# Amandaynzhou/CGC-Net

Measured on AMD Instinct MI355X. Metric: cell-graphs/sec (fwd+bwd), batch=32, ~1800 nodes/16 feat, higher is better.
Workload: dtype f32

## Files before the change

cgc-net_amd/csrc/rowops.hip:

```cpp
#include <type_traits>

#include "common.hpp"
#include "groups.hpp"

#define L2_EPS 1e-12f
#define RENORM_EPS 1e-15f
#define MAX_SLOTS 1024

template <int VEC, int MAXJ, int NQ>
__device__ __forceinline__ void col_reduce_store(float (&acc)[NQ][MAXJ][VEC], int F, int lpr, float* smem, float* slot) {
  const int lane = threadIdx.x & 63, wave = threadIdx.x >> 6;
#pragma unroll
  for (int q = 0; q < NQ; ++q)
#pragma unroll
    for (int j = 0; j < MAXJ; ++j)
#pragma unroll
      for (int v = 0; v < VEC; ++v)
        for (int o = 32; o >= lpr; o >>= 1) acc[q][j][v] += __shfl_xor(acc[q][j][v], o);
  if (wave > 0 && lane < lpr) {
#pragma unroll
    for (int q = 0; q < NQ; ++q)
#pragma unroll
      for (int j = 0; j < MAXJ; ++j)
#pragma unroll
        for (int v = 0; v < VEC; ++v) {
          const int c = (lane + lpr * j) * VEC + v;
          if (c < F) smem[((wave - 1) * NQ + q) * F + c] = acc[q][j][v];
        }
  }
  __syncthreads();
  if (wave == 0 && lane < lpr) {
#pragma unroll
    for (int q = 0; q < NQ; ++q)
#pragma unroll
      for (int j = 0; j < MAXJ; ++j)
#pragma unroll
        for (int v = 0; v < VEC; ++v) {
          const int c = (lane + lpr * j) * VEC + v;
          if (c < F) {
            float t = acc[q][j][v];
            for (int w = 0; w < 3; ++w) t += smem[(w * NQ + q) * F + c];
            slot[q * F + c] = t;
          }
        }
  }
}

template <int VEC, int MAXJ>
__device__ __forceinline__ void col_reduce_store_f64(double (&acc)[2][MAXJ][VEC], int F, int lpr, double* smem, double* slot) {
  const int lane = threadIdx.x & 63, wave = threadIdx.x >> 6;
#pragma unroll
  for (int q = 0; q < 2; ++q) {
#pragma unroll
    for (int j = 0; j < MAXJ; ++j)
#pragma unroll
      for (int v = 0; v < VEC; ++v)
        for (int o = 32; o >= lpr; o >>= 1) acc[q][j][v] += __shfl_xor(acc[q][j][v], o);
    if (q > 0) __syncthreads();
    if (wave > 0 && lane < lpr) {
#pragma unroll
      for (int j = 0; j < MAXJ; ++j)
#pragma unroll
        for (int v = 0; v < VEC; ++v) {
          const int c = (lane + lpr * j) * VEC + v;
          if (c < F) smem[(wave - 1) * F + c] = acc[q][j][v];
        }
    }
    __syncthreads();
    if (wave == 0 && lane < lpr) {
#pragma unroll
      for (int j = 0; j < MAXJ; ++j)
#pragma unroll
        for (int v = 0; v < VEC; ++v) {
          const int c = (lane + lpr * j) * VEC + v;
          if (c < F) {
            double t = acc[q][j][v];
            for (int w = 0; w < 3; ++w) t += smem[w * F + c];
            slot[q * F + c] = t;
          }
        }
    }
  }
}

#define RS_GROUPS 32
template <typename OUT, typename IN = float>
__global__ __launch_bounds__(32 * RS_GROUPS) void k_reduce_slots(const IN* __restrict__ ws, int slots, int width, OUT* __restrict__ out) {
  __shared__ double part[RS_GROUPS][32];
  const int cl = threadIdx.x & 31, grp = threadIdx.x >> 5;
  const int c = blockIdx.x * 32 + cl;
  double s = 0.0;
  if (c < width) {
    double a[4] = {0.0, 0.0, 0.0, 0.0};
    int k = grp;
    for (; k + 3 * RS_GROUPS < slots; k += 4 * RS_GROUPS) {
#pragma unroll
      for (int u = 0; u < 4; ++u) a[u] += (double)ws[(size_t)(k + RS_GROUPS * u) * width + c];
    }
    for (; k < slots; k += RS_GROUPS) a[0] += (double)ws[(size_t)k * width + c];
    s = (a[0] + a[1]) + (a[2] + a[3]);
  }
  part[grp][cl] = s;
  __syncthreads();
  if (grp == 0 && c < width) {
    double t[4] = {0.0, 0.0, 0.0, 0.0};
#pragma unroll
    for (int g = 0; g < RS_GROUPS; g += 4) { t[0] += part[g][cl]; t[1] += part[g + 1][cl]; t[2] += part[g + 2][cl]; t[3] += part[g + 3][cl]; }
    out[c] = (OUT)((t[0] + t[1]) + (t[2] + t[3]));
  }
}
#define REDUCE_SLOTS_GRID(width) dim3(ceil_div((width), 32))

__global__ __launch_bounds__(32 * RS_GROUPS) void k_reduce_slots_pair(const float* __restrict__ ws0, float* __restrict__ out0,
                                                                     const float* __restrict__ ws1, float* __restrict__ out1, int slots, int width) {
  const float* __restrict__ ws = blockIdx.y ? ws1 : ws0;
  float* __restrict__ out = blockIdx.y ? out1 : out0;
  __shared__ double part[RS_GROUPS][32];
  const int cl = threadIdx.x & 31, grp = threadIdx.x >> 5;
  const int c = blockIdx.x * 32 + cl;
  double s = 0.0;
  if (c < width) {
    double a[4] = {0.0, 0.0, 0.0, 0.0};
    int k = grp;
    for (; k + 3 * RS_GROUPS < slots; k += 4 * RS_GROUPS) {
#pragma unroll
      for (int u = 0; u < 4; ++u) a[u] += (double)ws[(size_t)(k + RS_GROUPS * u) * width + c];
    }
    for (; k < slots; k += RS_GROUPS) a[0] += (double)ws[(size_t)k * width + c];
    s = (a[0] + a[1]) + (a[2] + a[3]);
  }
  part[grp][cl] = s;
  __syncthreads();
  if (grp == 0 && c < width) {
    double t[4] = {0.0, 0.0, 0.0, 0.0};
#pragma unroll
    for (int g = 0; g < RS_GROUPS; g += 4) { t[0] += part[g][cl]; t[1] += part[g + 1][cl]; t[2] += part[g + 2][cl]; t[3] += part[g + 3][cl]; }
    out[c] = (float)((t[0] + t[1]) + (t[2] + t[3]));
  }
}
int launch_reduce_slots_f32_pair(const float* ws0, float* out0, const float* ws1, float* out1, int ng, int slots, int width, hipStream_t stream) {
  hipLaunchKernelGGL(k_reduce_slots_pair, dim3(ceil_div(width, 32), ng), dim3(32 * RS_GROUPS), 0, stream, ws0, out0, ws1, out1, slots, width);
  CGC_RETURN_IF_LAUNCH_FAILED();
  return 0;
}

int launch_reduce_slots_f32(const float* ws, int slots, int width, float* out, hipStream_t stream) {
  hipLaunchKernelGGL(k_reduce_slots<float>, REDUCE_SLOTS_GRID(width), dim3(32 * RS_GROUPS), 0, stream, ws, slots, width, out);
  CGC_RETURN_IF_LAUNCH_FAILED();
  return 0;
}

struct ColCfg {
  int vec, maxj, lpr, blocks;
  bool ok;
};
static ColCfg col_cfg(int n, int F, bool vec_ok) {
  ColCfg c;
  c.vec = vec_ok ? 4 : 1;
  c.ok = true;
  int chunks = F / c.vec;
  if (chunks <= 64) {
    c.maxj = 1;
    c.lpr = pick_lpr(chunks);
  } else {
    c.lpr = 64;
    int need = ceil_div(chunks, 64);
    if (c.vec == 4 && need > 8) {
      c.vec = 1;
      need = ceil_div(F, 64);
    }
    c.ok = need <= 32;
    c.maxj = need <= 2 ? 2 : need <= 4 ? 4 : (need == 5 && c.vec == 4) ? 5 : need <= 8 ? 8 : need <= 16 ? 16 : 32;
  }
  c.blocks = row_blocks(n, c.lpr, MAX_SLOTS);
  return c;
}

#define DISPATCH_COL(KERNEL, cfg, smem_bytes, stream, ...)                                                   \
  do {                                                                                                       \
    dim3 g__((cfg).blocks), b__(CGC_BLOCK);                                                                  \
    if ((cfg).vec == 4) {                                                                                    \
      switch ((cfg).maxj) {                                                                                  \
        case 1: hipLaunchKernelGGL((KERNEL<4, 1>), g__, b__, smem_bytes, stream, __VA_ARGS__); break;        \
        case 2: hipLaunchKernelGGL((KERNEL<4, 2>), g__, b__, smem_bytes, stream, __VA_ARGS__); break;        \
        case 4: hipLaunchKernelGGL((KERNEL<4, 4>), g__, b__, smem_bytes, stream, __VA_ARGS__); break;        \
        case 5: hipLaunchKernelGGL((KERNEL<4, 5>), g__, b__, smem_bytes, stream, __VA_ARGS__); break;        \
        default: hipLaunchKernelGGL((KERNEL<4, 8>), g__, b__, smem_bytes, stream, __VA_ARGS__); break;       \
      }                                                                                                      \
    } else {                                                                                                 \
      switch ((cfg).maxj) {                                                                                  \
        case 1: hipLaunchKernelGGL((KERNEL<1, 1>), g__, b__, smem_bytes, stream, __VA_ARGS__); break;        \
        case 2: hipLaunchKernelGGL((KERNEL<1, 2>), g__, b__, smem_bytes, stream, __VA_ARGS__); break;        \
        case 4: hipLaunchKernelGGL((KERNEL<1, 4>), g__, b__, smem_bytes, stream, __VA_ARGS__); break;        \
        case 8: hipLaunchKernelGGL((KERNEL<1, 8>), g__, b__, smem_bytes, stream, __VA_ARGS__); break;        \
        case 16: hipLaunchKernelGGL((KERNEL<1, 16>), g__, b__, smem_bytes, stream, __VA_ARGS__); break;      \
        default: hipLaunchKernelGGL((KERNEL<1, 32>), g__, b__, smem_bytes, stream, __VA_ARGS__); break;      \
      }                                                                                                      \
    }                                                                                                        \
  } while (0)

#define DISPATCH_COL_Y(KERNEL, cfg, ny, smem_bytes, stream, ...)                                                   \
  do {                                                                                                       \
    dim3 g__((cfg).blocks, (ny)), b__(CGC_BLOCK);                                                                    \
    if ((cfg).vec == 4) {                                                                                    \
      switch ((cfg).maxj) {                                                                                  \
        case 1: hipLaunchKernelGGL((KERNEL<4, 1>), g__, b__, smem_bytes, stream, __VA_ARGS__); break;        \
        case 2: hipLaunchKernelGGL((KERNEL<4, 2>), g__, b__, smem_bytes, stream, __VA_ARGS__); break;        \
        case 4: hipLaunchKernelGGL((KERNEL<4, 4>), g__, b__, smem_bytes, stream, __VA_ARGS__); break;        \
        case 5: hipLaunchKernelGGL((KERNEL<4, 5>), g__, b__, smem_bytes, stream, __VA_ARGS__); break;        \
        default: hipLaunchKernelGGL((KERNEL<4, 8>), g__, b__, smem_bytes, stream, __VA_ARGS__); break;       \
      }                                                                                                      \
    } else {                                                                                                 \
      switch ((cfg).maxj) {                                                                                  \
        case 1: hipLaunchKernelGGL((KERNEL<1, 1>), g__, b__, smem_bytes, stream, __VA_ARGS__); break;        \
        case 2: hipLaunchKernelGGL((KERNEL<1, 2>), g__, b__, smem_bytes, stream, __VA_ARGS__); break;        \
        case 4: hipLaunchKernelGGL((KERNEL<1, 4>), g__, b__, smem_bytes, stream, __VA_ARGS__); break;        \
        case 8: hipLaunchKernelGGL((KERNEL<1, 8>), g__, b__, smem_bytes, stream, __VA_ARGS__); break;        \
        case 16: hipLaunchKernelGGL((KERNEL<1, 16>), g__, b__, smem_bytes, stream, __VA_ARGS__); break;      \
        default: hipLaunchKernelGGL((KERNEL<1, 32>), g__, b__, smem_bytes, stream, __VA_ARGS__); break;      \
      }                                                                                                      \
    }                                                                                                        \
  } while (0)


extern "C" int cgc_stats_blocks(int n, int F) {
  (void)F;
  int b = ceil_div(n > 0 ? n : 1, 4);
  return b < MAX_SLOTS ? b : MAX_SLOTS;
}
extern "C" int64_t cgc_stats_ws_floats(int n, int F) {
  const int b = cgc_stats_blocks(n, F);
  return (int64_t)(b > 1 ? b : 1) * 4 * F + 4 * (int64_t)F + 2;
}

template <int VEC, int MAXJ>
__global__ __launch_bounds__(256) void k_l2norm_act_stats(const float* __restrict__ h, int n, int F, int lpr, int normalize,
                                                          int act, float* __restrict__ hn, float* __restrict__ rinv,
                                                          float* __restrict__ ws) {
  extern __shared__ __attribute__((aligned(16))) float smem[];
  const RowGroup rg(lpr);
  double acc[2][MAXJ][VEC];
#pragma unroll
  for (int j = 0; j < MAXJ; ++j)
#pragma unroll
    for (int v = 0; v < VEC; ++v) acc[0][j][v] = acc[1][j][v] = 0.0;

  for (int base = rg.gwave * rg.rpw; base < n; base += rg.nwaves * rg.rpw) {
    const int row = base + rg.sub;
    const bool valid = row < n;
    Vec<VEC> x[MAXJ];
    float ss = 0.f;
#pragma unroll
    for (int j = 0; j < MAXJ; ++j) {
      const int c = (rg.sl + lpr * j) * VEC;
      if (valid && c < F) {
        load_wide<VEC, MAXJ>(x[j], h + (size_t)row * F + c);
#pragma unroll
        for (int v = 0; v < VEC; ++v) ss += x[j].v[v] * x[j].v[v];
      } else {
#pragma unroll
        for (int v = 0; v < VEC; ++v) x[j].v[v] = 0.f;
      }
    }
    ss = group_sum(ss, lpr);
    const float r = normalize ? 1.f / fmaxf(sqrtf(ss), L2_EPS) : 1.f;
#pragma unroll
    for (int j = 0; j < MAXJ; ++j) {
      const int c = (rg.sl + lpr * j) * VEC;
      if (valid && c < F) {
#pragma unroll
        for (int v = 0; v < VEC; ++v) {
          x[j].v[v] *= r;
          const double o = (double)act_fwd(x[j].v[v], act);
          acc[0][j][v] += o;
          acc[1][j][v] = fma(o, o, acc[1][j][v]);
        }
        x[j].store(hn + (size_t)row * F + c);
      }
    }
    if (valid && rg.sl == 0) rinv[row] = r;
  }
  if (ws != nullptr)
    col_reduce_store_f64<VEC, MAXJ>(acc, F, lpr, reinterpret_cast<double*>(smem), reinterpret_cast<double*>(ws) + (size_t)blockIdx.x * 2 * F);
}

extern "C" int cgc_l2norm_act_stats(const float* h, int n, int F, int normalize, int act, float* hn, float* rinv,
                                    double* stats, float* ws, cgc_stream_t stream) {
  if (n <= 0 || F <= 0) {
    if (stats && F > 0) (void)hipMemsetAsync(stats, 0, sizeof(double) * 2 * F, as_stream(stream));
    return 0;
  }
  const bool vec_ok = (F % 4 == 0) && aligned16(h) && aligned16(hn);
  ColCfg cfg = col_cfg(n, F, vec_ok);
  if (!cfg.ok) return CGC_EINVAL;
  float* wsp = stats ? ws : nullptr;
  if (stats && !ws) return CGC_EINVAL;
  const size_t smem = sizeof(float) * 3 * 2 * F;
  DISPATCH_COL(k_l2norm_act_stats, cfg, smem, as_stream(stream), h, n, F, cfg.lpr, normalize, act, hn, rinv, wsp);
  CGC_RETURN_IF_LAUNCH_FAILED();
  if (stats) {
    hipLaunchKernelGGL((k_reduce_slots<double, double>), REDUCE_SLOTS_GRID(2 * F), dim3(32 * RS_GROUPS), 0, as_stream(stream),
                       reinterpret_cast<const double*>(ws), cfg.blocks, 2 * F, stats);
    CGC_RETURN_IF_LAUNCH_FAILED();
  }
  return 0;
}

__global__ void k_bn_finalize(const double* __restrict__ stats, int F, double count, float eps, float momentum,
                              float* running_mean, float* running_var, float* __restrict__ mean, float* __restrict__ istd,
                              long long* nbt) {
  const int f = blockIdx.x * blockDim.x + threadIdx.x;
  if (f == 0 && nbt != nullptr) *nbt += 1;
  if (f >= F) return;
  const double m = stats[f] / count;
  double var = stats[F + f] / count - m * m;
  if (var < 0.0) var = 0.0;
  mean[f] = (float)m;
  istd[f] = (float)(1.0 / sqrt(var + (double)eps));
  if (running_mean != nullptr) {
    const double unbiased = var * count / (count > 1.0 ? count - 1.0 : 1.0);
    running_mean[f] = (1.f - momentum) * running_mean[f] + momentum * (float)m;
    running_var[f] = (1.f - momentum) * running_var[f] + momentum * (float)unbiased;
  }
}

extern "C" int cgc_bn_finalize(const double* stats, int F, double count, float eps, float momentum, float* running_mean,
                               float* running_var, float* mean, float* istd, cgc_stream_t stream) {
  if (F <= 0) return 0;
  hipLaunchKernelGGL(k_bn_finalize, dim3(ceil_div(F, 256)), dim3(256), 0, as_stream(stream), stats, F, count, eps, momentum,
                     running_mean, running_var, mean, istd, (long long*)nullptr);
  CGC_RETURN_IF_LAUNCH_FAILED();
  return 0;
}

__global__ void k_bn_running_stats(const float* __restrict__ rm, const float* __restrict__ rv, int F, float eps, float* __restrict__ mean,
                                   float* __restrict__ istd) {
  const int f = blockIdx.x * blockDim.x + threadIdx.x;
  if (f >= F) return;
  mean[f] = rm[f];
  istd[f] = 1.f / sqrtf(rv[f] + eps);
}
extern "C" int cgc_bn_running_stats(const float* running_mean, const float* running_var, int F, float eps, float* mean, float* istd,
                                    cgc_stream_t stream) {
  if (F <= 0) return 0;
  if (running_mean == nullptr || running_var == nullptr || mean == nullptr || istd == nullptr) return CGC_EINVAL;
  hipLaunchKernelGGL(k_bn_running_stats, dim3(ceil_div(F, 256)), dim3(256), 0, as_stream(stream), running_mean, running_var, F, eps, mean, istd);
  CGC_RETURN_IF_LAUNCH_FAILED();
  return 0;
}

__global__ __launch_bounds__(32 * RS_GROUPS) void k_stats_finalize(const StatsFinPtrs p0, const StatsFinPtrs p1, int slots, int F, double count) {
  const StatsFinPtrs& p = blockIdx.y ? p1 : p0;
  const double* __restrict__ ws = reinterpret_cast<const double*>(p.ws);
  const float eps = p.eps, momentum = p.momentum;
  float* running_mean = p.running_mean;
  float* running_var = p.running_var;
  float* __restrict__ mean = p.mean;
  float* __restrict__ istd = p.istd;
  long long* nbt = p.nbt;
  __shared__ double part[2][RS_GROUPS][32];
  const int cl = threadIdx.x & 31, grp = threadIdx.x >> 5;
  const int f = blockIdx.x * 32 + cl;
  if (blockIdx.x == 0 && threadIdx.x == 0 && nbt != nullptr) *nbt += 1;
#pragma unroll
  for (int q = 0; q < 2; ++q) {
    double s = 0.0;
    if (f < F) {
      const double* col = ws + (size_t)q * F + f;
      const size_t width = 2 * (size_t)F;
      double a[4] = {0.0, 0.0, 0.0, 0.0};
      int k = grp;
      for (; k + 3 * RS_GROUPS < slots; k += 4 * RS_GROUPS) {
#pragma unroll
        for (int u = 0; u < 4; ++u) a[u] += col[(size_t)(k + RS_GROUPS * u) * width];
      }
      for (; k < slots; k += RS_GROUPS) a[0] += col[(size_t)k * width];
      s = (a[0] + a[1]) + (a[2] + a[3]);
    }
    part[q][grp][cl] = s;
  }
  __syncthreads();
  if (grp != 0 || f >= F) return;
  double t0[4] = {0.0, 0.0, 0.0, 0.0}, t1[4] = {0.0, 0.0, 0.0, 0.0};
#pragma unroll
  for (int g = 0; g < RS_GROUPS; g += 4)
#pragma unroll
    for (int u = 0; u < 4; ++u) { t0[u] += part[0][g + u][cl]; t1[u] += part[1][g + u][cl]; }
  const double s0 = (t0[0] + t0[1]) + (t0[2] + t0[3]), s1 = (t1[0] + t1[1]) + (t1[2] + t1[3]);
  const double m = s0 / count;
  double var = s1 / count - m * m;
  if (var < 0.0) var = 0.0;
  mean[f] = (float)m;
  istd[f] = (float)(1.0 / sqrt(var + (double)eps));
  if (running_mean != nullptr) {
    const double unbiased = var * count / (count > 1.0 ? count - 1.0 : 1.0);
    running_mean[f] = (1.f - momentum) * running_mean[f] + momentum * (float)m;
    running_var[f] = (1.f - momentum) * running_var[f] + momentum * (float)unbiased;
  }
}

int launch_stats_finalize_groups(const StatsFinPtrs* g, int ng, int slots, int F, double count, hipStream_t stream) {
  hipLaunchKernelGGL(k_stats_finalize, dim3(ceil_div(F, 32), ng), dim3(32 * RS_GROUPS), 0, stream, g[0], g[ng - 1], slots, F, count);
  CGC_RETURN_IF_LAUNCH_FAILED();
  return 0;
}
int launch_stats_finalize(const float* ws, int slots, int F, double count, float eps, float momentum, float* running_mean,
                          float* running_var, float* mean, float* istd, int64_t* nbt, hipStream_t stream) {
  const StatsFinPtrs g{ws, running_mean, running_var, mean, istd, reinterpret_cast<long long*>(nbt), eps, momentum};
  return launch_stats_finalize_groups(&g, 1, slots, F, count, stream);
}

extern "C" int cgc_l2norm_act_bn(const float* h, int n, int F, int normalize, int act, float* hn, float* rinv, float* ws,
                                 double count, float eps, float momentum, float* running_mean, float* running_var,
                                 int64_t* num_batches_tracked, float* mean, float* istd, cgc_stream_t stream) {
  if (F <= 0) return 0;
  if (ws == nullptr || mean == nullptr || istd == nullptr) return CGC_EINVAL;
  int slots = 0;
  if (n > 0) {
    const bool vec_ok = (F % 4 == 0) && aligned16(h) && aligned16(hn);
    ColCfg cfg = col_cfg(n, F, vec_ok);
    if (!cfg.ok) return CGC_EINVAL;
    const size_t smem = sizeof(float) * 3 * 2 * F;
    DISPATCH_COL(k_l2norm_act_stats, cfg, smem, as_stream(stream), h, n, F, cfg.lpr, normalize, act, hn, rinv, ws);
    CGC_RETURN_IF_LAUNCH_FAILED();
    slots = cfg.blocks;
  }
  return launch_stats_finalize(ws, slots, F, count, eps, momentum, running_mean, running_var, mean, istd, num_batches_tracked, as_stream(stream));
}

template <int VEC, int MAXJ>
__global__ __launch_bounds__(256) void k_bn_act_apply(const BnApplyPtrs p0, const BnApplyPtrs p1, int n, int F, int lpr, int act, int ldy) {
  const BnApplyPtrs& p = blockIdx.y ? p1 : p0;
  const float* __restrict__ hn = p.hn;
  const float* __restrict__ mean = p.mean;
  const float* __restrict__ istd = p.istd;
  const float* __restrict__ gamma = p.gamma;
  const float* __restrict__ beta = p.beta;
  float* __restrict__ y = p.y;
  float* __restrict__ y2 = p.y2;
  const int ldy2 = p.ldy2;
  const RowGroup rg(lpr);
  float mu[MAXJ][VEC], sc[MAXJ][VEC], sh[MAXJ][VEC];
#pragma unroll
  for (int j = 0; j < MAXJ; ++j)
#pragma unroll
    for (int v = 0; v < VEC; ++v) {
      mu[j][v] = 0.f;
      sc[j][v] = 1.f;
      sh[j][v] = 0.f;
    }
  if (mean != nullptr) {
#pragma unroll
    for (int j = 0; j < MAXJ; ++j)
#pragma unroll
      for (int v = 0; v < VEC; ++v) {
        const int c = min((rg.sl + lpr * j) * VEC + v, F - 1);
        mu[j][v] = mean[c];
        sc[j][v] = istd[c] * gamma[c];
        sh[j][v] = beta[c];
      }
  }
  auto rows = [&](auto act_c) {
    constexpr int ACT = decltype(act_c)::value;
    const int last = F - VEC;
    for (int base = rg.gwave * rg.rpw; base < n; base += rg.nwaves * rg.rpw) {
      const int row = base + rg.sub;
      const bool rowok = row < n;
      Vec<VEC> x[MAXJ];
#pragma unroll
      for (int j = 0; j < MAXJ; ++j) load_wide<VEC, MAXJ>(x[j], hn + (size_t)min(row, n - 1) * F + min((rg.sl + lpr * j) * VEC, last));
#pragma unroll
      for (int j = 0; j < MAXJ; ++j) {
        const int c = (rg.sl + lpr * j) * VEC;
#pragma unroll
        for (int v = 0; v < VEC; ++v) x[j].v[v] = fmaf(act_fwd(x[j].v[v], ACT) - mu[j][v], sc[j][v], sh[j][v]);
        if (rowok && c < F) {
          x[j].store(y + (size_t)row * ldy + c);
          if (y2 != nullptr) x[j].store(y2 + (size_t)row * ldy2 + c);
        }
      }
    }
  };
  switch (act) {
    case CGC_ACT_RELU: rows(std::integral_constant<int, CGC_ACT_RELU>()); break;
    case CGC_ACT_ELU: rows(std::integral_constant<int, CGC_ACT_ELU>()); break;
    case CGC_ACT_LEAKYRELU: rows(std::integral_constant<int, CGC_ACT_LEAKYRELU>()); break;
    default: rows(std::integral_constant<int, CGC_ACT_IDENTITY>()); break;
  }
}

int bn_act_apply_groups(const BnApplyPtrs* g, int ng, int n, int F, int act, int ldy, hipStream_t stream) {
  if (n <= 0 || F <= 0) return 0;
  if (ng < 1 || ng > 2) return CGC_EINVAL;
  bool vec = (F % 4 == 0) && (ldy % 4 == 0);
  for (int i = 0; i < ng; ++i)
    vec = vec && aligned16(g[i].hn) && aligned16(g[i].y) && (g[i].y2 == nullptr || (g[i].ldy2 % 4 == 0 && aligned16(g[i].y2)));
  ColCfg cfg = col_cfg(n, F, vec);
  if (!cfg.ok) return CGC_EINVAL;
  cfg.blocks = row_blocks(n, cfg.lpr, 1024);
  DISPATCH_COL_Y(k_bn_act_apply, cfg, ng, 0, stream, g[0], g[ng - 1], n, F, cfg.lpr, act, ldy);
  CGC_RETURN_IF_LAUNCH_FAILED();
  return 0;
}
extern "C" int cgc_bn_act_apply(const float* hn, int n, int F, int act, const float* mean, const float* istd, const float* gamma,
                                const float* beta, float* y, int ldy, float* y2, int ldy2, cgc_stream_t stream) {
  const BnApplyPtrs g{hn, mean, istd, gamma, beta, y, y2, ldy2};
  return bn_act_apply_groups(&g, 1, n, F, act, ldy, as_stream(stream));
}

template <int VEC, int MAXJ>
__global__ __launch_bounds__(256) void k_bn_bwd_reduce(const BnRedPtrs p0, const BnRedPtrs p1, int ldy, int n, int F, int lpr, int act) {
  const BnRedPtrs& p = blockIdx.y ? p1 : p0;
  const float* __restrict__ dy = p.dy;
  const float* __restrict__ hn = p.hn;
  const float* __restrict__ mean = p.mean;
  const float* __restrict__ istd = p.istd;
  float* __restrict__ ws = p.ws;
  extern __shared__ __attribute__((aligned(16))) float smem[];
  const RowGroup rg(lpr);
  float acc[2][MAXJ][VEC];
  float mu[MAXJ][VEC], is[MAXJ][VEC];
#pragma unroll
  for (int j = 0; j < MAXJ; ++j)
#pragma unroll
    for (int v = 0; v < VEC; ++v) {
      acc[0][j][v] = acc[1][j][v] = 0.f;
      const int c = min((rg.sl + lpr * j) * VEC + v, F - 1);
      mu[j][v] = mean[c];
      is[j][v] = istd[c];
    }
  for (int base = rg.gwave * rg.rpw; base < n; base += rg.nwaves * rg.rpw) {
    const int row = base + rg.sub;
    if (row < n) {
#pragma unroll
      for (int j = 0; j < MAXJ; ++j) {
        const int c = (rg.sl + lpr * j) * VEC;
        if (c < F) {
          Vec<VEC> d, x;
          load_wide<VEC, MAXJ>(d, dy + (size_t)row * ldy + c);
          load_wide<VEC, MAXJ>(x, hn + (size_t)row * F + c);
#pragma unroll
          for (int v = 0; v < VEC; ++v) {
            const float xhat = (act_fwd(x.v[v], act) - mu[j][v]) * is[j][v];
            acc[0][j][v] += d.v[v];
            acc[1][j][v] += d.v[v] * xhat;
          }
        }
      }
    }
  }
  col_reduce_store<VEC, MAXJ, 2>(acc, F, lpr, smem, ws + (size_t)blockIdx.x * 2 * F);
}

int bn_bwd_reduce_groups(const BnRedPtrs* g, float* const* sums, int ng, int ldy, int n, int F, int act, hipStream_t stream) {
  if (F <= 0) return 0;
  if (ng < 1 || ng > 2) return CGC_EINVAL;
  if (n <= 0) {
    for (int i = 0; i < ng; ++i) (void)hipMemsetAsync(sums[i], 0, sizeof(float) * 2 * F, stream);
    return 0;
  }
  bool vec_ok = (F % 4 == 0) && (ldy % 4 == 0);
  for (int i = 0; i < ng; ++i) vec_ok = vec_ok && aligned16(g[i].dy) && aligned16(g[i].hn);
  ColCfg cfg = col_cfg(n, F, vec_ok);
  if (!cfg.ok) return CGC_EINVAL;
  const size_t smem = sizeof(float) * 3 * 2 * F;
  DISPATCH_COL_Y(k_bn_bwd_reduce, cfg, ng, smem, stream, g[0], g[ng - 1], ldy, n, F, cfg.lpr, act);
  CGC_RETURN_IF_LAUNCH_FAILED();
  return launch_reduce_slots_f32_pair(g[0].ws, sums[0], g[ng - 1].ws, sums[ng - 1], ng, cfg.blocks, 2 * F, stream);
}
extern "C" int cgc_bn_bwd_reduce(const float* dy, int ldy, const float* hn, int n, int F, int act, const float* mean,
                                 const float* istd, float* sums, float* ws, cgc_stream_t stream) {
  const BnRedPtrs g{dy, hn, mean, istd, ws};
  float* const out[1] = {sums};
  return bn_bwd_reduce_groups(&g, out, 1, ldy, n, F, act, as_stream(stream));
}

template <int VEC, int MAXJ>
__global__ __launch_bounds__(256) void k_bn_act_l2_bwd(const float* __restrict__ dy, int ldy, const float* __restrict__ hn,
                                                       const float* __restrict__ rinv, int n, int F, int lpr, int act,
                                                       int normalize, int mode, const float* __restrict__ mean,
                                                       const float* __restrict__ istd, const float* __restrict__ gamma,
                                                       const float* __restrict__ sums, float inv_count, float* __restrict__ dh,
                                                       float* __restrict__ ws ) {
  extern __shared__ __attribute__((aligned(16))) float smem[];
  const RowGroup rg(lpr);
  float csum[1][MAXJ][VEC];
#pragma unroll
  for (int j = 0; j < MAXJ; ++j)
#pragma unroll
    for (int v = 0; v < VEC; ++v) csum[0][j][v] = 0.f;
  constexpr bool REGC = MAXJ * VEC <= 8;
  constexpr int RJ = REGC ? MAXJ : 1, RV = REGC ? VEC : 1;
  float ca[RJ][RV], cb[RJ][RV], cc[RJ][RV], mu[RJ][RV], is[RJ][RV];
  if (REGC) {
#pragma unroll
    for (int j = 0; j < RJ; ++j)
#pragma unroll
      for (int v = 0; v < RV; ++v) {
        const int c = (rg.sl + lpr * j) * VEC + v;
        ca[j][v] = 1.f; cb[j][v] = cc[j][v] = mu[j][v] = is[j][v] = 0.f;
        if (mode != 0 && c < F) {
          ca[j][v] = gamma[c] * istd[c];
          if (mode == 2) {
            cb[j][v] = ca[j][v] * sums[c] * inv_count;
            cc[j][v] = ca[j][v] * sums[F + c] * inv_count;
            mu[j][v] = mean[c];
            is[j][v] = istd[c];
          }
        }
      }
  }
  float* const lc = smem + 3 * (size_t)F;
  if (!REGC && mode != 0) {
    for (int c = threadIdx.x; c < F; c += blockDim.x) {
      const float a_ = gamma[c] * istd[c];
      lc[c] = a_;
      lc[F + c] = mode == 2 ? a_ * sums[c] * inv_count : 0.f;
      lc[2 * F + c] = mode == 2 ? a_ * sums[F + c] * inv_count : 0.f;
      lc[3 * F + c] = mode == 2 ? mean[c] : 0.f;
      lc[4 * F + c] = mode == 2 ? istd[c] : 0.f;
    }
    __syncthreads();
  }
  auto rows = [&](auto act_c, auto hot_c) {
    constexpr int ACT = decltype(act_c)::value;
    constexpr bool HOT = decltype(hot_c)::value;
    const int mode_rt = mode, normalize_rt = normalize;
    const int mode = HOT ? 2 : mode_rt;
    const int normalize = HOT ? 1 : normalize_rt;
    for (int base = rg.gwave * rg.rpw; base < n; base += rg.nwaves * rg.rpw) {
      const int row = min(base + rg.sub, n - 1);
      const bool valid = base + rg.sub < n;
      Vec<VEC> g[MAXJ], x[MAXJ];
      float dot = 0.f;
  #pragma unroll
      for (int j = 0; j < MAXJ; ++j) {
        const int c = min((rg.sl + lpr * j) * VEC, F - VEC);
        load_wide<VEC, MAXJ>(g[j], dy + (size_t)row * ldy + c);
        load_wide<VEC, MAXJ>(x[j], hn + (size_t)row * F + c);
      }
  #pragma unroll
      for (int j = 0; j < MAXJ; ++j) {
        const int c = (rg.sl + lpr * j) * VEC;
        if (valid && c < F) {
          Vec<VEC> pa, pb, pc, pm, pi;
          if (!REGC && mode != 0) {
            pa.load(lc + c);
            if (mode == 2) { pb.load(lc + F + c); pc.load(lc + 2 * F + c); pm.load(lc + 3 * F + c); pi.load(lc + 4 * F + c); }
          }
  #pragma unroll
          for (int v = 0; v < VEC; ++v) {
            const float xv = x[j].v[v];
            float a_, b_ = 0.f, c_ = 0.f, m_ = 0.f, i_ = 0.f;
            if (REGC) {
              a_ = ca[REGC ? j : 0][REGC ? v : 0]; b_ = cb[REGC ? j : 0][REGC ? v : 0]; c_ = cc[REGC ? j : 0][REGC ? v : 0];
              m_ = mu[REGC ? j : 0][REGC ? v : 0]; i_ = is[REGC ? j : 0][REGC ? v : 0];
            } else if (mode != 0) {
              a_ = pa.v[v];
              if (mode == 2) { b_ = pb.v[v]; c_ = pc.v[v]; m_ = pm.v[v]; i_ = pi.v[v]; }
            } else {
              a_ = 1.f;
            }
            float go = a_ * g[j].v[v];
            if (mode == 2) go = go - b_ - (act_fwd(xv, ACT) - m_) * i_ * c_;
            go *= act_bwd(xv, ACT);
            g[j].v[v] = go;
            dot += xv * go;
          }
        } else {
  #pragma unroll
          for (int v = 0; v < VEC; ++v) g[j].v[v] = x[j].v[v] = 0.f;
        }
      }
      if (normalize) dot = group_sum(dot, lpr);
      if (!valid) continue;
      const float r = normalize ? rinv[row] : 1.f;
      const bool clamped = normalize && !(r < 1.f / L2_EPS);
  #pragma unroll
      for (int j = 0; j < MAXJ; ++j) {
        const int c = (rg.sl + lpr * j) * VEC;
        if (c < F) {
          Vec<VEC> o;
  #pragma unroll
          for (int v = 0; v < VEC; ++v) {
            const float gv = g[j].v[v];
            o.v[v] = !normalize ? gv : (clamped ? gv * (1.f / L2_EPS) : r * (gv - x[j].v[v] * dot));
            csum[0][j][v] += o.v[v];
          }
          o.store(dh + (size_t)row * F + c);
        }
      }
    }
  };
  if (mode == 2 && normalize) {
    switch (act) {
      case CGC_ACT_RELU: rows(std::integral_constant<int, CGC_ACT_RELU>(), std::true_type()); break;
      case CGC_ACT_ELU: rows(std::integral_constant<int, CGC_ACT_ELU>(), std::true_type()); break;
      case CGC_ACT_LEAKYRELU: rows(std::integral_constant<int, CGC_ACT_LEAKYRELU>(), std::true_type()); break;
      default: rows(std::integral_constant<int, CGC_ACT_IDENTITY>(), std::true_type()); break;
    }
  } else {
    switch (act) {
      case CGC_ACT_RELU: rows(std::integral_constant<int, CGC_ACT_RELU>(), std::false_type()); break;
      case CGC_ACT_ELU: rows(std::integral_constant<int, CGC_ACT_ELU>(), std::false_type()); break;
      case CGC_ACT_LEAKYRELU: rows(std::integral_constant<int, CGC_ACT_LEAKYRELU>(), std::false_type()); break;
      default: rows(std::integral_constant<int, CGC_ACT_IDENTITY>(), std::false_type()); break;
    }
  }
  if (ws != nullptr) col_reduce_store<VEC, MAXJ, 1>(csum, F, lpr, smem, ws + (size_t)blockIdx.x * F);
}

extern "C" int cgc_bn_act_l2_bwd(const float* dy, int ldy, const float* hn, const float* rinv, int n, int F, int act,
                                 int normalize, int mode, const float* mean, const float* istd, const float* gamma,
                                 const float* sums, double count, float* dh, float* dh_colsum, float* ws, cgc_stream_t stream) {
  if (F <= 0) return 0;
  if (n <= 0) {
    if (dh_colsum) (void)hipMemsetAsync(dh_colsum, 0, sizeof(float) * F, as_stream(stream));
    return 0;
  }
  if (dh_colsum != nullptr && ws == nullptr) return CGC_EINVAL;
  const bool vec = (F % 4 == 0) && (ldy % 4 == 0) && aligned16(dy) && aligned16(hn) && aligned16(dh);
  ColCfg cfg = col_cfg(n, F, vec);
  if (!cfg.ok) return CGC_EINVAL;
  if (dh_colsum == nullptr) cfg.blocks = row_blocks(n, cfg.lpr);
  const float inv_count = (float)(1.0 / count);
  const size_t smem = sizeof(float) * (3 + 5) * F;
  DISPATCH_COL(k_bn_act_l2_bwd, cfg, smem, as_stream(stream), dy, ldy, hn, rinv, n, F, cfg.lpr, act, normalize, mode, mean, istd,
               gamma, sums, inv_count, dh, dh_colsum ? ws : (float*)nullptr);
  CGC_RETURN_IF_LAUNCH_FAILED();
  if (dh_colsum) {
    hipLaunchKernelGGL(k_reduce_slots<float>, REDUCE_SLOTS_GRID(F), dim3(32 * RS_GROUPS), 0, as_stream(stream), ws, cfg.blocks, F, dh_colsum);
    CGC_RETURN_IF_LAUNCH_FAILED();
  }
  return 0;
}

template <int VEC, int MAXJ>
__global__ __launch_bounds__(256) void k_colsum(const float* __restrict__ x, int ld, int n, int F, int lpr, float* __restrict__ ws) {
  extern __shared__ __attribute__((aligned(16))) float smem[];
  const RowGroup rg(lpr);
  float acc[1][MAXJ][VEC];
#pragma unroll
  for (int j = 0; j < MAXJ; ++j)
#pragma unroll
    for (int v = 0; v < VEC; ++v) acc[0][j][v] = 0.f;
  for (int base = rg.gwave * rg.rpw; base < n; base += rg.nwaves * rg.rpw) {
    const int row = base + rg.sub;
    if (row < n) {
#pragma unroll
      for (int j = 0; j < MAXJ; ++j) {
        const int c = (rg.sl + lpr * j) * VEC;
        if (c < F) {
          Vec<VEC> d;
          d.load(x + (size_t)row * ld + c);
#pragma unroll
          for (int v = 0; v < VEC; ++v) acc[0][j][v] += d.v[v];
        }
      }
    }
  }
  col_reduce_store<VEC, MAXJ, 1>(acc, F, lpr, smem, ws + (size_t)blockIdx.x * F);
}

extern "C" int cgc_colsum(const float* x, int ld, int n, int F, float* out, float* ws, cgc_stream_t stream) {
  if (F <= 0) return 0;
  if (n <= 0) {
    (void)hipMemsetAsync(out, 0, sizeof(float) * F, as_stream(stream));
    return 0;
  }
  const bool vec_ok = (F % 4 == 0) && (ld % 4 == 0) && aligned16(x);
  ColCfg cfg = col_cfg(n, F, vec_ok);
  if (!cfg.ok) return CGC_EINVAL;
  const size_t smem = sizeof(float) * 3 * F;
  DISPATCH_COL(k_colsum, cfg, smem, as_stream(stream), x, ld, n, F, cfg.lpr, ws);
  CGC_RETURN_IF_LAUNCH_FAILED();
  hipLaunchKernelGGL(k_reduce_slots<float>, REDUCE_SLOTS_GRID(F), dim3(32 * RS_GROUPS), 0, as_stream(stream), ws, cfg.blocks, F, out);
  CGC_RETURN_IF_LAUNCH_FAILED();
  return 0;
}

template <int VEC>
__global__ __launch_bounds__(256) void k_softmax_fwd(const float* __restrict__ x, int n, int C, int ld, int lpr, float* __restrict__ out) {
  const RowGroup rg(lpr);
  for (int base = rg.gwave * rg.rpw; base < n; base += rg.nwaves * rg.rpw) {
    const int row = base + rg.sub;
    const bool valid = row < n;
    const float* xr = x + (size_t)row * ld;
    float m = -INFINITY;
    if (valid)
      for (int c = rg.sl * VEC; c < C; c += lpr * VEC) {
        Vec<VEC> t;
        t.load(xr + c);
#pragma unroll
        for (int v = 0; v < VEC; ++v) m = fmaxf(m, t.v[v]);
      }
    m = group_max(m, lpr);
    float s = 0.f;
    if (valid)
      for (int c = rg.sl * VEC; c < C; c += lpr * VEC) {
        Vec<VEC> t;
        t.load(xr + c);
#pragma unroll
        for (int v = 0; v < VEC; ++v) s += expf(t.v[v] - m);
      }
    s = group_sum(s, lpr);
    if (!valid) continue;
    const float inv = 1.f / s;
    for (int c = rg.sl * VEC; c < C; c += lpr * VEC) {
      Vec<VEC> t;
      t.load(xr + c);
#pragma unroll
      for (int v = 0; v < VEC; ++v) t.v[v] = expf(t.v[v] - m) * inv;
      t.store(out + (size_t)row * ld + c);
    }
  }
}

template <int VEC, int MAXJ>
__global__ __launch_bounds__(256) void k_softmax_fwd_reg(const float* __restrict__ x, int n, int C, int ld, int lpr,
                                                         float* __restrict__ out) {
  const RowGroup rg(lpr);
  for (int base = rg.gwave * rg.rpw; base < n; base += rg.nwaves * rg.rpw) {
    const int row = base + rg.sub;
    const bool valid = row < n;
    const float* xr = x + (size_t)row * ld;
    Vec<VEC> t[MAXJ];
    float m = -INFINITY;
#pragma unroll
    for (int j = 0; j < MAXJ; ++j) {
      const int c = (rg.sl + lpr * j) * VEC;
      if (valid && c < C) {
        t[j].load(xr + c);
#pragma unroll
        for (int v = 0; v < VEC; ++v) m = fmaxf(m, t[j].v[v]);
      }
    }
    m = group_max(m, lpr);
    float s = 0.f;
#pragma unroll
    for (int j = 0; j < MAXJ; ++j) {
      const int c = (rg.sl + lpr * j) * VEC;
      if (valid && c < C) {
#pragma unroll
        for (int v = 0; v < VEC; ++v) {
          t[j].v[v] = expf(t[j].v[v] - m);
          s += t[j].v[v];
        }
      }
    }
    s = group_sum(s, lpr);
    if (!valid) continue;
    const float inv = 1.f / s;
#pragma unroll
    for (int j = 0; j < MAXJ; ++j) {
      const int c = (rg.sl + lpr * j) * VEC;
      if (c < C) {
#pragma unroll
        for (int v = 0; v < VEC; ++v) t[j].v[v] *= inv;
        t[j].store(out + (size_t)row * ld + c);
      }
    }
  }
}

template <int VEC, int MAXJ>
__global__ __launch_bounds__(256) void k_softmax_bwd(const float* __restrict__ S, const float* __restrict__ dS, int n, int C,
                                                     int ld, int lpr, float* __restrict__ dx, float* __restrict__ ws) {
  extern __shared__ __attribute__((aligned(16))) float smem[];
  const RowGroup rg(lpr);
  float csum[1][MAXJ][VEC];
#pragma unroll
  for (int j = 0; j < MAXJ; ++j)
#pragma unroll
    for (int v = 0; v < VEC; ++v) csum[0][j][v] = 0.f;
  for (int base = rg.gwave * rg.rpw; base < n; base += rg.nwaves * rg.rpw) {
    const int row = min(base + rg.sub, n - 1);
    const bool valid = base + rg.sub < n;
    Vec<VEC> s[MAXJ], d[MAXJ];
    float dot = 0.f;
#pragma unroll
    for (int j = 0; j < MAXJ; ++j) {
      const int c = min((rg.sl + lpr * j) * VEC, C - VEC);
      load_wide<VEC, MAXJ>(s[j], S + (size_t)row * ld + c);
      load_wide<VEC, MAXJ>(d[j], dS + (size_t)row * ld + c);
    }
#pragma unroll
    for (int j = 0; j < MAXJ; ++j) {
      const bool ok = valid && (rg.sl + lpr * j) * VEC < C;
#pragma unroll
      for (int v = 0; v < VEC; ++v) {
        s[j].v[v] = ok ? s[j].v[v] : 0.f;
        d[j].v[v] = ok ? d[j].v[v] : 0.f;
        dot += s[j].v[v] * d[j].v[v];
      }
    }
    dot = group_sum(dot, lpr);
    if (!valid) continue;
#pragma unroll
    for (int j = 0; j < MAXJ; ++j) {
      const int c = (rg.sl + lpr * j) * VEC;
      if (c < C) {
#pragma unroll
        for (int v = 0; v < VEC; ++v) {
          d[j].v[v] = s[j].v[v] * (d[j].v[v] - dot);
          csum[0][j][v] += d[j].v[v];
        }
        d[j].store(dx + (size_t)row * ld + c);
      }
    }
  }
  if (ws != nullptr) col_reduce_store<VEC, MAXJ, 1>(csum, C, lpr, smem, ws + (size_t)blockIdx.x * C);
}

extern "C" int cgc_softmax_fwd(const float* x, int n, int C, int ld, float* out, cgc_stream_t stream) {
  if (n <= 0 || C <= 0) return 0;
  if (ld < C) return CGC_EINVAL;
  const bool vec = (C % 4 == 0) && (ld % 4 == 0) && aligned16(x) && aligned16(out);
  ColCfg cfg = col_cfg(n, C, vec);
  if (cfg.ok && cfg.maxj <= 8) {
    cfg.blocks = row_blocks(n, cfg.lpr);
    DISPATCH_COL(k_softmax_fwd_reg, cfg, 0, as_stream(stream), x, n, C, ld, cfg.lpr, out);
    CGC_RETURN_IF_LAUNCH_FAILED();
    return 0;
  }
  const int lpr = pick_lpr(vec ? C / 4 : C);
  dim3 grid(row_blocks(n, lpr)), block(CGC_BLOCK);
  if (vec)
    hipLaunchKernelGGL(k_softmax_fwd<4>, grid, block, 0, as_stream(stream), x, n, C, ld, lpr, out);
  else
    hipLaunchKernelGGL(k_softmax_fwd<1>, grid, block, 0, as_stream(stream), x, n, C, ld, lpr, out);
  CGC_RETURN_IF_LAUNCH_FAILED();
  return 0;
}

extern "C" int cgc_softmax_bwd(const float* S, const float* dS, int n, int C, int ld, float* dx, float* dx_colsum, float* ws,
                               cgc_stream_t stream) {
  if (C <= 0) return 0;
  if (ld < C) return CGC_EINVAL;
  if (n <= 0) {
    if (dx_colsum) (void)hipMemsetAsync(dx_colsum, 0, sizeof(float) * C, as_stream(stream));
    return 0;
  }
  if (dx_colsum != nullptr && ws == nullptr) return CGC_EINVAL;
  const bool vec = (C % 4 == 0) && (ld % 4 == 0) && aligned16(S) && aligned16(dS) && aligned16(dx);
  ColCfg cfg = col_cfg(n, C, vec);
  if (!cfg.ok) return CGC_EINVAL;
  if (dx_colsum == nullptr) cfg.blocks = row_blocks(n, cfg.lpr);
  const size_t smem = dx_colsum ? sizeof(float) * 3 * C : 0;
  DISPATCH_COL(k_softmax_bwd, cfg, smem, as_stream(stream), S, dS, n, C, ld, cfg.lpr, dx, dx_colsum ? ws : (float*)nullptr);
  CGC_RETURN_IF_LAUNCH_FAILED();
  if (dx_colsum) {
    hipLaunchKernelGGL(k_reduce_slots<float>, REDUCE_SLOTS_GRID(C), dim3(32 * RS_GROUPS), 0, as_stream(stream), ws, cfg.blocks, C, dx_colsum);
    CGC_RETURN_IF_LAUNCH_FAILED();
  }
  return 0;
}

#define SEGMAX_WAVES 16
__global__ __launch_bounds__(64 * SEGMAX_WAVES) void k_segment_max_fwd(const float* __restrict__ x, const int* __restrict__ gptr,
                                                                       int D, int nmax, float* __restrict__ out,
                                                                       int* __restrict__ arg) {
  __shared__ float bv[SEGMAX_WAVES][64];
  __shared__ int bi[SEGMAX_WAVES][64];
  const int b = blockIdx.x;
  const int lane = threadIdx.x & 63, wave = threadIdx.x >> 6;
  int dp = 64;
  if (D <= 32) dp = D <= 2 ? 2 : D <= 4 ? 4 : D <= 8 ? 8 : D <= 16 ? 16 : 32;
  const int rpw = 64 / dp, sub = lane / dp, dl = lane - sub * dp;
  const int d = blockIdx.y * 64 + dl;
  const int lo = gptr[b], hi = gptr[b + 1];
  float best = -INFINITY;
  int idx = -1;
  if (d < D) {
    const int stride = SEGMAX_WAVES * rpw;
    int r = lo + wave * rpw + sub;
    for (; r + 3 * stride < hi; r += 4 * stride) {
      float v[4];
#pragma unroll
      for (int u = 0; u < 4; ++u) v[u] = x[(size_t)(r + u * stride) * D + d];
#pragma unroll
      for (int u = 0; u < 4; ++u)
        if (v[u] > best) { best = v[u]; idx = r + u * stride; }
    }
    for (; r < hi; r += stride) {
      const float v = x[(size_t)r * D + d];
      if (v > best) { best = v; idx = r; }
    }
  }
  bv[wave][lane] = best;
  bi[wave][lane] = idx;
  __syncthreads();
  if (wave == 0 && sub == 0 && d < D) {
    for (int w = 0; w < SEGMAX_WAVES; ++w)
      for (int s2 = (w == 0 ? 1 : 0); s2 < rpw; ++s2) {
        const float v = bv[w][s2 * dp + dl];
        const int i = bi[w][s2 * dp + dl];
        if (i >= 0 && (v > best || (v == best && i < idx) || idx < 0)) { best = v; idx = i; }
      }
    if (idx < 0) { best = 0.f; }
    else if (hi - lo < nmax && best < 0.f) { best = 0.f; idx = -1; }
    out[(size_t)b * D + d] = best;
    arg[(size_t)b * D + d] = idx;
  }
}

__global__ void k_segment_max_bwd(const float* __restrict__ dout, const int* __restrict__ arg, int total, int D, float* __restrict__ dx) {
  const int i = blockIdx.x * blockDim.x + threadIdx.x;
  if (i >= total) return;
  const int a = arg[i];
  if (a >= 0) dx[(size_t)a * D + (i % D)] = dout[i];
}

extern "C" int cgc_segment_max_fwd(const float* x, const int* gptr, int B, int D, int nmax, float* out, int* arg, cgc_stream_t stream) {
  if (B <= 0 || D <= 0) return 0;
  hipLaunchKernelGGL(k_segment_max_fwd, dim3(B, ceil_div(D, 64)), dim3(64 * SEGMAX_WAVES), 0, as_stream(stream), x, gptr, D, nmax, out, arg);
  CGC_RETURN_IF_LAUNCH_FAILED();
  return 0;
}

__global__ void k_segment_max_bwd_full(const float* __restrict__ dout, const int* __restrict__ arg, const int* __restrict__ gptr, int D,
                                       float* __restrict__ dx) {
  const int b = blockIdx.y;
  const int g0 = gptr[b], cnt = (gptr[b + 1] - g0) * D;
  for (int i = blockIdx.x * blockDim.x + threadIdx.x; i < cnt; i += gridDim.x * blockDim.x) {
    const int r = i / D, d = i - r * D;
    dx[(size_t)g0 * D + i] = (arg[b * D + d] == g0 + r) ? dout[b * D + d] : 0.f;
  }
}

extern "C" int cgc_segment_max_bwd_full(const float* dout, const int* arg, const int* gptr, int B, int D, int nmax, float* dx,
                                        cgc_stream_t stream) {
  if (B <= 0 || D <= 0 || nmax <= 0) return 0;
  if (B > 65535) return CGC_EINVAL;
  int bx = ceil_div(nmax * D, 256 * 4);
  if (bx < 1) bx = 1;
  hipLaunchKernelGGL(k_segment_max_bwd_full, dim3(bx, B), dim3(256), 0, as_stream(stream), dout, arg, gptr, D, dx);
  CGC_RETURN_IF_LAUNCH_FAILED();
  return 0;
}

extern "C" int cgc_segment_max_bwd(const float* dout, const int* arg, int B, int D, float* dx_zeroed, cgc_stream_t stream) {
  if (B <= 0 || D <= 0) return 0;
  const int total = B * D;
  hipLaunchKernelGGL(k_segment_max_bwd, dim3(ceil_div(total, 256)), dim3(256), 0, as_stream(stream), dout, arg, total, D, dx_zeroed);
  CGC_RETURN_IF_LAUNCH_FAILED();
  return 0;
}

template <int VEC>
__global__ __launch_bounds__(256) void k_dense_rownorm_fwd(const float* __restrict__ A, int R, int C, int lpr, float* __restrict__ out,
                                                           float* __restrict__ invd, float* __restrict__ ge1) {
  const RowGroup rg(lpr);
  for (int base = rg.gwave * rg.rpw; base < R; base += rg.nwaves * rg.rpw) {
    const int row = base + rg.sub;
    const bool valid = row < R;
    float s = 0.f;
    if (valid)
      for (int c = rg.sl * VEC; c < C; c += lpr * VEC) {
        Vec<VEC> t;
        t.load(A + (size_t)row * C + c);
#pragma unroll
        for (int v = 0; v < VEC; ++v) s += t.v[v];
      }
    s = group_sum(s, lpr);
    if (!valid) continue;
    const float inv = 1.f / fmaxf(s, 1.f);
    for (int c = rg.sl * VEC; c < C; c += lpr * VEC) {
      Vec<VEC> t;
      t.load(A + (size_t)row * C + c);
#pragma unroll
      for (int v = 0; v < VEC; ++v) t.v[v] *= inv;
      t.store(out + (size_t)row * C + c);
    }
    if (rg.sl == 0) {
      invd[row] = inv;
      ge1[row] = s >= 1.f ? 1.f : 0.f;
    }
  }
}

template <int VEC>
__global__ __launch_bounds__(256) void k_dense_rownorm_bwd(const float* __restrict__ dOut, const float* __restrict__ An,
                                                           const float* __restrict__ invd, const float* __restrict__ ge1, int R, int C,
                                                           int lpr, float* __restrict__ dA) {
  const RowGroup rg(lpr);
  for (int base = rg.gwave * rg.rpw; base < R; base += rg.nwaves * rg.rpw) {
    const int row = base + rg.sub;
    const bool valid = row < R;
    float t = 0.f;
    if (valid)
      for (int c = rg.sl * VEC; c < C; c += lpr * VEC) {
        Vec<VEC> g, a;
        g.load(dOut + (size_t)row * C + c);
        a.load(An + (size_t)row * C + c);
#pragma unroll
        for (int v = 0; v < VEC; ++v) t += g.v[v] * a.v[v];
      }
    t = group_sum(t, lpr);
    if (!valid) continue;
    const float inv = invd[row], sub = ge1[row] * t;
    for (int c = rg.sl * VEC; c < C; c += lpr * VEC) {
      Vec<VEC> g;
      g.load(dOut + (size_t)row * C + c);
#pragma unroll
      for (int v = 0; v < VEC; ++v) g.v[v] = inv * (g.v[v] - sub);
      g.store(dA + (size_t)row * C + c);
    }
  }
}

template <int VEC>
__global__ __launch_bounds__(256) void k_dense_renorm_fwd(const float* __restrict__ A, int R, int C, int lpr, float p, float* __restrict__ out) {
  const RowGroup rg(lpr);
  const float omp = 1.f - p;
  for (int base = rg.gwave * rg.rpw; base < R; base += rg.nwaves * rg.rpw) {
    const int row = base + rg.sub;
    const bool valid = row < R;
    const int diag = valid ? row % C : -1;
    float s = 0.f;
    if (valid)
      for (int c = rg.sl * VEC; c < C; c += lpr * VEC) {
        Vec<VEC> t;
        t.load(A + (size_t)row * C + c);
#pragma unroll
        for (int v = 0; v < VEC; ++v) s += (c + v == diag) ? 0.f : t.v[v];
      }
    s = group_sum(s, lpr);
    if (!valid) continue;
    const float den = s + RENORM_EPS;
    for (int c = rg.sl * VEC; c < C; c += lpr * VEC) {
      Vec<VEC> t;
      t.load(A + (size_t)row * C + c);
#pragma unroll
      for (int v = 0; v < VEC; ++v) t.v[v] = (c + v == diag) ? p : (t.v[v] / den) * omp;
      t.store(out + (size_t)row * C + c);
    }
  }
}

template <int VEC>
__global__ __launch_bounds__(256) void k_dense_renorm_bwd(const float* __restrict__ A, const float* __restrict__ dOut, int R, int C,
                                                          int lpr, float p, float* __restrict__ dA) {
  const RowGroup rg(lpr);
  const float omp = 1.f - p;
  for (int base = rg.gwave * rg.rpw; base < R; base += rg.nwaves * rg.rpw) {
    const int row = base + rg.sub;
    const bool valid = row < R;
    const int diag = valid ? row % C : -1;
    float s = 0.f, t = 0.f;
    if (valid)
      for (int c = rg.sl * VEC; c < C; c += lpr * VEC) {
        Vec<VEC> a, g;
        a.load(A + (size_t)row * C + c);
        g.load(dOut + (size_t)row * C + c);
#pragma unroll
        for (int v = 0; v < VEC; ++v)
          if (c + v != diag) { s += a.v[v]; t += a.v[v] * g.v[v]; }
      }
    s = group_sum(s, lpr);
    t = group_sum(t, lpr);
    if (!valid) continue;
    const float q = 1.f / (s + RENORM_EPS);
    for (int c = rg.sl * VEC; c < C; c += lpr * VEC) {
      Vec<VEC> g;
      g.load(dOut + (size_t)row * C + c);
#pragma unroll
      for (int v = 0; v < VEC; ++v) g.v[v] = (c + v == diag) ? 0.f : omp * q * (g.v[v] - q * t);
      g.store(dA + (size_t)row * C + c);
    }
  }
}

template <int VEC>
__global__ __launch_bounds__(256) void k_adj_prep_fwd(const float* __restrict__ A, int R, int C, int lpr, float p, float* __restrict__ At,
                                                      float* __restrict__ An, float* __restrict__ invd, float* __restrict__ ge1) {
  const RowGroup rg(lpr);
  const bool renorm = p >= 0.f;
  const float omp = 1.f - p;
  for (int base = rg.gwave * rg.rpw; base < R; base += rg.nwaves * rg.rpw) {
    const int row = base + rg.sub;
    const bool valid = row < R;
    const int diag = (valid && renorm) ? row % C : -1;
    float s = 0.f;
    if (valid)
      for (int c = rg.sl * VEC; c < C; c += lpr * VEC) {
        Vec<VEC> t;
        t.load(A + (size_t)row * C + c);
#pragma unroll
        for (int v = 0; v < VEC; ++v) s += (c + v == diag) ? 0.f : t.v[v];
      }
    s = group_sum(s, lpr);
    float st = s;
    const float den = s + RENORM_EPS;
    if (renorm) {
      st = 0.f;
      if (valid)
        for (int c = rg.sl * VEC; c < C; c += lpr * VEC) {
          Vec<VEC> t;
          t.load(A + (size_t)row * C + c);
#pragma unroll
          for (int v = 0; v < VEC; ++v) { t.v[v] = (c + v == diag) ? p : (t.v[v] / den) * omp; st += t.v[v]; }
          t.store(At + (size_t)row * C + c);
        }
      st = group_sum(st, lpr);
    }
    if (!valid) continue;
    const float inv = 1.f / fmaxf(st, 1.f);
    for (int c = rg.sl * VEC; c < C; c += lpr * VEC) {
      Vec<VEC> t;
      t.load(A + (size_t)row * C + c);
#pragma unroll
      for (int v = 0; v < VEC; ++v) {
        const float at = renorm ? ((c + v == diag) ? p : (t.v[v] / den) * omp) : t.v[v];
        t.v[v] = at * inv;
      }
      t.store(An + (size_t)row * C + c);
    }
    if (rg.sl == 0) {
      invd[row] = inv;
      ge1[row] = st >= 1.f ? 1.f : 0.f;
    }
  }
}

template <int VEC>
__global__ __launch_bounds__(256) void k_adj_prep_bwd(const float* __restrict__ A, const float* __restrict__ An, const float* __restrict__ invd,
                                                      const float* __restrict__ ge1, const float* __restrict__ gAn,
                                                      const float* __restrict__ gAt, int R, int C, int lpr, float p, float* __restrict__ dA) {
  const RowGroup rg(lpr);
  const bool renorm = p >= 0.f;
  const float omp = 1.f - p;
  for (int base = rg.gwave * rg.rpw; base < R; base += rg.nwaves * rg.rpw) {
    const int row = base + rg.sub;
    const bool valid = row < R;
    const int diag = (valid && renorm) ? row % C : -1;
    float t1 = 0.f, s = 0.f, u = 0.f, w = 0.f;
    if (valid)
      for (int c = rg.sl * VEC; c < C; c += lpr * VEC) {
        Vec<VEC> g, an, a, h;
        g.load(gAn + (size_t)row * C + c);
        an.load(An + (size_t)row * C + c);
#pragma unroll
        for (int v = 0; v < VEC; ++v) t1 += g.v[v] * an.v[v];
        if (renorm) {
          a.load(A + (size_t)row * C + c);
          if (gAt != nullptr) h.load(gAt + (size_t)row * C + c);
#pragma unroll
          for (int v = 0; v < VEC; ++v)
            if (c + v != diag) { s += a.v[v]; u += a.v[v] * g.v[v]; if (gAt != nullptr) w += a.v[v] * h.v[v]; }
        }
      }
    t1 = group_sum(t1, lpr);
    if (renorm) { s = group_sum(s, lpr); u = group_sum(u, lpr); w = group_sum(w, lpr); }
    if (!valid) continue;
    const float inv = invd[row], sub = ge1[row] * t1;
    const float q = 1.f / (s + RENORM_EPS);
    const float t = inv * (u - sub * s) + w;
    for (int c = rg.sl * VEC; c < C; c += lpr * VEC) {
      Vec<VEC> g, h;
      g.load(gAn + (size_t)row * C + c);
      if (gAt != nullptr) h.load(gAt + (size_t)row * C + c);
#pragma unroll
      for (int v = 0; v < VEC; ++v) {
        float d = inv * (g.v[v] - sub);
        if (gAt != nullptr) d += h.v[v];
        g.v[v] = renorm ? ((c + v == diag) ? 0.f : omp * q * (d - q * t)) : d;
      }
      g.store(dA + (size_t)row * C + c);
    }
  }
}

template <int VEC, int MAXJ>
__global__ __launch_bounds__(256) void k_adj_prep_fwd_reg(const float* __restrict__ A, int R, int C, int lpr, float p, float* __restrict__ At,
                                                          float* __restrict__ An, float* __restrict__ invd, float* __restrict__ ge1) {
  const RowGroup rg(lpr);
  const bool renorm = p >= 0.f;
  const float omp = 1.f - p;
  for (int base = rg.gwave * rg.rpw; base < R; base += rg.nwaves * rg.rpw) {
    const int row = base + rg.sub;
    const bool valid = row < R;
    const int diag = (valid && renorm) ? row % C : -1;
    Vec<VEC> t[MAXJ];
    float s = 0.f;
#pragma unroll
    for (int j = 0; j < MAXJ; ++j) {
      const int c = (rg.sl + lpr * j) * VEC;
      if (valid && c < C) {
        t[j].load(A + (size_t)row * C + c);
#pragma unroll
        for (int v = 0; v < VEC; ++v) s += (c + v == diag) ? 0.f : t[j].v[v];
      }
    }
    s = group_sum(s, lpr);
    float st = s;
    const float den = s + RENORM_EPS;
    if (renorm) {
      st = 0.f;
#pragma unroll
      for (int j = 0; j < MAXJ; ++j) {
        const int c = (rg.sl + lpr * j) * VEC;
        if (valid && c < C) {
#pragma unroll
          for (int v = 0; v < VEC; ++v) { t[j].v[v] = (c + v == diag) ? p : (t[j].v[v] / den) * omp; st += t[j].v[v]; }
          t[j].store(At + (size_t)row * C + c);
        }
      }
      st = group_sum(st, lpr);
    }
    if (!valid) continue;
    const float inv = 1.f / fmaxf(st, 1.f);
#pragma unroll
    for (int j = 0; j < MAXJ; ++j) {
      const int c = (rg.sl + lpr * j) * VEC;
      if (c < C) {
#pragma unroll
        for (int v = 0; v < VEC; ++v) t[j].v[v] *= inv;
        t[j].store(An + (size_t)row * C + c);
      }
    }
    if (rg.sl == 0) {
      invd[row] = inv;
      ge1[row] = st >= 1.f ? 1.f : 0.f;
    }
  }
}

template <int VEC, int MAXJ>
__global__ __launch_bounds__(256) void k_adj_prep_bwd_reg(const float* __restrict__ A, const float* __restrict__ An,
                                                          const float* __restrict__ invd, const float* __restrict__ ge1,
                                                          const float* __restrict__ gAn, const float* __restrict__ gAt, int R, int C,
                                                          int lpr, float p, float* __restrict__ dA) {
  const RowGroup rg(lpr);
  const bool renorm = p >= 0.f;
  const float omp = 1.f - p;
  for (int base = rg.gwave * rg.rpw; base < R; base += rg.nwaves * rg.rpw) {
    const int row = base + rg.sub;
    const bool valid = row < R;
    const int diag = (valid && renorm) ? row % C : -1;
    float t1 = 0.f, s = 0.f, u = 0.f, w = 0.f;
    Vec<VEC> g[MAXJ], h[MAXJ];
    if (renorm) {
      Vec<VEC> a[MAXJ];
#pragma unroll
      for (int j = 0; j < MAXJ; ++j) {
        const int c = (rg.sl + lpr * j) * VEC;
        if (valid && c < C) {
          load_wide<VEC, MAXJ>(g[j], gAn + (size_t)row * C + c);
          load_wide<VEC, MAXJ>(a[j], A + (size_t)row * C + c);
          if (gAt != nullptr) load_wide<VEC, MAXJ>(h[j], gAt + (size_t)row * C + c);
#pragma unroll
          for (int v = 0; v < VEC; ++v) s += (c + v == diag) ? 0.f : a[j].v[v];
        }
      }
      s = group_sum(s, lpr);
      const float den = s + RENORM_EPS, inv_f = valid ? invd[row] : 0.f;
#pragma unroll
      for (int j = 0; j < MAXJ; ++j) {
        const int c = (rg.sl + lpr * j) * VEC;
        if (valid && c < C) {
#pragma unroll
          for (int v = 0; v < VEC; ++v) {
            const bool dg = c + v == diag;
            const float at = dg ? p : (a[j].v[v] / den) * omp;
            t1 += g[j].v[v] * (at * inv_f);
            if (!dg) { u += a[j].v[v] * g[j].v[v]; if (gAt != nullptr) w += a[j].v[v] * h[j].v[v]; }
          }
        }
      }
    } else {
#pragma unroll
      for (int j = 0; j < MAXJ; ++j) {
        const int c = (rg.sl + lpr * j) * VEC;
        if (valid && c < C) {
          Vec<VEC> an;
          load_wide<VEC, MAXJ>(g[j], gAn + (size_t)row * C + c);
          load_wide<VEC, MAXJ>(an, An + (size_t)row * C + c);
#pragma unroll
          for (int v = 0; v < VEC; ++v) t1 += g[j].v[v] * an.v[v];
          if (gAt != nullptr) load_wide<VEC, MAXJ>(h[j], gAt + (size_t)row * C + c);
        }
      }
    }
    t1 = group_sum(t1, lpr);
    if (renorm) { u = group_sum(u, lpr); w = group_sum(w, lpr); }
    if (!valid) continue;
    const float inv = invd[row], sub = ge1[row] * t1;
    const float q = 1.f / (s + RENORM_EPS);
    const float t = inv * (u - sub * s) + w;
#pragma unroll
    for (int j = 0; j < MAXJ; ++j) {
      const int c = (rg.sl + lpr * j) * VEC;
      if (c < C) {
#pragma unroll
        for (int v = 0; v < VEC; ++v) {
          float d = inv * (g[j].v[v] - sub);
          if (gAt != nullptr) d += h[j].v[v];
          g[j].v[v] = renorm ? ((c + v == diag) ? 0.f : omp * q * (d - q * t)) : d;
        }
        g[j].store(dA + (size_t)row * C + c);
      }
    }
  }
}

#define LAUNCH_ROW(KERNEL, vec, lpr, R, stream, ...)                                                          \
  do {                                                                                                        \
    dim3 g__(row_blocks(R, lpr)), b__(CGC_BLOCK);                                                             \
    if (vec) hipLaunchKernelGGL(KERNEL<4>, g__, b__, 0, stream, __VA_ARGS__);                                 \
    else hipLaunchKernelGGL(KERNEL<1>, g__, b__, 0, stream, __VA_ARGS__);                                     \
  } while (0)

extern "C" int cgc_dense_rownorm_fwd(const float* A, int R, int C, float* out, float* invd, float* ge1, cgc_stream_t stream) {
  if (R <= 0 || C <= 0) return 0;
  const bool vec = (C % 4 == 0) && aligned16(A) && aligned16(out);
  const int lpr = pick_lpr(vec ? C / 4 : C);
  LAUNCH_ROW(k_dense_rownorm_fwd, vec, lpr, R, as_stream(stream), A, R, C, lpr, out, invd, ge1);
  CGC_RETURN_IF_LAUNCH_FAILED();
  return 0;
}
extern "C" int cgc_dense_rownorm_bwd(const float* dOut, const float* Anorm, const float* invd, const float* ge1, int R, int C,
                                     float* dA, cgc_stream_t stream) {
  if (R <= 0 || C <= 0) return 0;
  const bool vec = (C % 4 == 0) && aligned16(dOut) && aligned16(Anorm) && aligned16(dA);
  const int lpr = pick_lpr(vec ? C / 4 : C);
  LAUNCH_ROW(k_dense_rownorm_bwd, vec, lpr, R, as_stream(stream), dOut, Anorm, invd, ge1, R, C, lpr, dA);
  CGC_RETURN_IF_LAUNCH_FAILED();
  return 0;
}
extern "C" int cgc_dense_renorm_fwd(const float* A, int R, int C, float p, float* out, cgc_stream_t stream) {
  if (R <= 0 || C <= 0) return 0;
  const bool vec = (C % 4 == 0) && aligned16(A) && aligned16(out);
  const int lpr = pick_lpr(vec ? C / 4 : C);
  LAUNCH_ROW(k_dense_renorm_fwd, vec, lpr, R, as_stream(stream), A, R, C, lpr, p, out);
  CGC_RETURN_IF_LAUNCH_FAILED();
  return 0;
}
extern "C" int cgc_dense_renorm_bwd(const float* A, const float* dOut, int R, int C, float p, float* dA, cgc_stream_t stream) {
  if (R <= 0 || C <= 0) return 0;
  const bool vec = (C % 4 == 0) && aligned16(A) && aligned16(dOut) && aligned16(dA);
  const int lpr = pick_lpr(vec ? C / 4 : C);
  LAUNCH_ROW(k_dense_renorm_bwd, vec, lpr, R, as_stream(stream), A, dOut, R, C, lpr, p, dA);
  CGC_RETURN_IF_LAUNCH_FAILED();
  return 0;
}

extern "C" int cgc_adj_prep_fwd(const float* A, int R, int C, float p, float* At, float* An, float* invd, float* ge1, cgc_stream_t stream) {
  if (R <= 0 || C <= 0) return 0;
  if (p >= 0.f && At == nullptr) return CGC_EINVAL;
  const bool vec = (C % 4 == 0) && aligned16(A) && aligned16(An) && (At == nullptr || aligned16(At));
  ColCfg cfg = col_cfg(R, C, vec);
  if (cfg.ok && cfg.maxj <= 8) {
    cfg.blocks = row_blocks(R, cfg.lpr);
    DISPATCH_COL(k_adj_prep_fwd_reg, cfg, 0, as_stream(stream), A, R, C, cfg.lpr, p, At, An, invd, ge1);
    CGC_RETURN_IF_LAUNCH_FAILED();
    return 0;
  }
  const int lpr = pick_lpr(vec ? C / 4 : C);
  LAUNCH_ROW(k_adj_prep_fwd, vec, lpr, R, as_stream(stream), A, R, C, lpr, p, At, An, invd, ge1);
  CGC_RETURN_IF_LAUNCH_FAILED();
  return 0;
}
extern "C" int cgc_adj_prep_bwd(const float* A, const float* An, const float* invd, const float* ge1, const float* gAn, const float* gAt,
                                int R, int C, float p, float* dA, cgc_stream_t stream) {
  if (R <= 0 || C <= 0) return 0;
  const bool vec = (C % 4 == 0) && aligned16(A) && aligned16(An) && aligned16(gAn) && aligned16(dA) && (gAt == nullptr || aligned16(gAt));
  ColCfg cfg = col_cfg(R, C, vec);
  if (cfg.ok && cfg.maxj <= 8) {
    cfg.blocks = row_blocks(R, cfg.lpr);
    DISPATCH_COL(k_adj_prep_bwd_reg, cfg, 0, as_stream(stream), A, An, invd, ge1, gAn, gAt, R, C, cfg.lpr, p, dA);
    CGC_RETURN_IF_LAUNCH_FAILED();
    return 0;
  }
  const int lpr = pick_lpr(vec ? C / 4 : C);
  LAUNCH_ROW(k_adj_prep_bwd, vec, lpr, R, as_stream(stream), A, An, invd, ge1, gAn, gAt, R, C, lpr, p, dA);
  CGC_RETURN_IF_LAUNCH_FAILED();
  return 0;
}
```

cgc-net_amd/csrc/sagenarrow.hip:

```cpp
#include "common.hpp"
#include "groups.hpp"

#define L2_EPS 1e-12f
typedef float floatx16 __attribute__((ext_vector_type(16)));

template <int CTRL>
__device__ __forceinline__ float dpp_step(float v) {
  return v + __builtin_bit_cast(float, __builtin_amdgcn_mov_dpp(__builtin_bit_cast(int, v), CTRL, 0xF, 0xF, true));
}
__device__ __forceinline__ float half_sum(float v) {
  v = dpp_step<0xB1>(v);
  v = dpp_step<0x4E>(v);
  v = dpp_step<0x141>(v);
  v = dpp_step<0x140>(v);
  return v + __shfl_xor(v, 16);
}

#define SN_LDT 33

template <int FS, int ACT>
__global__ __launch_bounds__(256) void k_sage_narrow_bwd(const SnBwdPtrs p0, const SnBwdPtrs p1, int ldy, int n, int F, int ,
                                                         int normalize, int mode, float inv_count, int lda, int fin, int ldd, int tiles) {
  const bool second = blockIdx.y != 0;
  const float* __restrict__ dy = second ? p1.dy : p0.dy;
  const float* __restrict__ hn = second ? p1.hn : p0.hn;
  const float* __restrict__ rinv = second ? p1.rinv : p0.rinv;
  const float* __restrict__ mean = second ? p1.mean : p0.mean;
  const float* __restrict__ istd = second ? p1.istd : p0.istd;
  const float* __restrict__ gamma = second ? p1.gamma : p0.gamma;
  const float* __restrict__ sums = second ? p1.sums : p0.sums;
  const float* __restrict__ agg = second ? p1.agg : p0.agg;
  const float* __restrict__ W = second ? p1.W : p0.W;
  float* __restrict__ dagg = second ? p1.dagg : p0.dagg;
  float* __restrict__ ws = second ? p1.ws : p0.ws;
  __shared__ float strip[4][17 * 64];
  const int lane = threadIdx.x & 63, wave = threadIdx.x >> 6;
  const int f = lane & 31, half = lane >> 5;
  const bool fok = f < F;
  float ca = 1.f, cb = 0.f, cc = 0.f, mu = 0.f, is = 0.f;
  if (mode != 0 && fok) {
    ca = gamma[f] * istd[f];
    if (mode == 2) {
      cb = ca * sums[f] * inv_count;
      cc = ca * sums[F + f] * inv_count;
      mu = mean[f];
      is = istd[f];
    }
  }
  float wb[FS];
#pragma unroll
  for (int t = 0; t < FS; ++t) {
    const int ff = 2 * t + half;
    wb[t] = (dagg != nullptr && f < fin && ff < F) ? W[(size_t)f * F + ff] : 0.f;
  }
  floatx16 dw;
#pragma unroll
  for (int r = 0; r < 16; ++r) dw[r] = 0.f;
  float db = 0.f;
  float* __restrict__ st = strip[wave];

  const int fcl = fok ? f : 0, facl = f < fin ? f : 0;
  for (int tile = blockIdx.x * 4 + wave; tile < tiles; tile += gridDim.x * 4) {
    const int row0 = tile * 32;
    float dh[16], ag[16];
#pragma unroll
    for (int s = 0; s < 16; ++s) {
      const int row = row0 + 2 * s + half;
      const bool ok = row < n;
      const size_t rc = ok ? row : n - 1;
      const float g_ = dy[rc * ldy + fcl], x_ = hn[rc * F + fcl], a_ = agg[rc * lda + facl];
      const float g = (ok && fok) ? g_ : 0.f;
      const float x = (ok && fok) ? x_ : 0.f;
      ag[s] = (ok && f < fin) ? a_ : 0.f;
      float go = ca * g;
      if (mode == 2) go = go - cb - (act_fwd(x, ACT) - mu) * is * cc;
      go *= act_bwd(x, ACT);
      if (!(ok && fok)) go = 0.f;
      float o = go;
      if (normalize) {
        const float dot = half_sum(x * go);
        const float r_ = rinv[rc];
        const float r = ok ? r_ : 1.f;
        const bool clamped = !(r < 1.f / L2_EPS);
        o = clamped ? go * (1.f / L2_EPS) : r * (go - x * dot);
      }
      dh[s] = o;
      db += o;
    }
#pragma unroll
    for (int s = 0; s < 16; ++s) dw = __builtin_amdgcn_mfma_f32_32x32x2f32(ag[s], dh[s], dw, 0, 0, 0);
    if (dagg != nullptr) {
#pragma unroll
      for (int s = 0; s < 16; ++s) st[(2 * s + half) * SN_LDT + f] = dh[s];
      __builtin_amdgcn_wave_barrier();
      floatx16 da;
#pragma unroll
      for (int r = 0; r < 16; ++r) da[r] = 0.f;
#pragma unroll
      for (int t = 0; t < FS; ++t) da = __builtin_amdgcn_mfma_f32_32x32x2f32(st[f * SN_LDT + 2 * t + half], wb[t], da, 0, 0, 0);
      __builtin_amdgcn_wave_barrier();
      if (f < fin) {
        if (row0 + 32 <= n) {
#pragma unroll
          for (int r = 0; r < 16; ++r) dagg[(size_t)(row0 + (r & 3) + 8 * (r >> 2) + 4 * half) * ldd + f] = da[r];
        } else {
#pragma unroll
          for (int r = 0; r < 16; ++r) {
            const int row = row0 + (r & 3) + 8 * (r >> 2) + 4 * half;
            if (row < n) dagg[(size_t)row * ldd + f] = da[r];
          }
        }
      }
    }
  }
  __syncthreads();
  float* __restrict__ xch = &strip[0][0];
  static_assert(32 * SN_LDT <= 17 * 64, "transposition strip exceeds the per-wave LDS");
#pragma unroll
  for (int r = 0; r < 16; ++r) xch[(wave * 17 + r) * 64 + lane] = dw[r];
  xch[(wave * 17 + 16) * 64 + lane] = db;
  __syncthreads();
  if (wave == 0) {
    float* __restrict__ slot = ws + (size_t)blockIdx.x * (fin * F + F);
#pragma unroll
    for (int r = 0; r < 16; ++r) {
      const float v = (xch[(0 * 17 + r) * 64 + lane] + xch[(1 * 17 + r) * 64 + lane]) + (xch[(2 * 17 + r) * 64 + lane] + xch[(3 * 17 + r) * 64 + lane]);
      const int k = (r & 3) + 8 * (r >> 2) + 4 * half;
      if (fok && k < fin) slot[k * F + f] = v;
    }
    float d = (xch[(0 * 17 + 16) * 64 + lane] + xch[(1 * 17 + 16) * 64 + lane]) + (xch[(2 * 17 + 16) * 64 + lane] + xch[(3 * 17 + 16) * 64 + lane]);
    d += __shfl_xor(d, 32);
    if (fok && half == 0) slot[fin * F + f] = d;
  }
}

int launch_reduce_slots_f32(const float* ws, int slots, int width, float* out, hipStream_t stream);

static int sn_grid(int n) {
  const int tiles = ceil_div(n, 32);
  int g = ceil_div(tiles, 4);
  return g < 1024 ? g : 1024;
}

extern "C" int64_t cgc_sage_narrow_ws_floats(int n, int fin, int F) { return (int64_t)sn_grid(n > 0 ? n : 1) * (fin * F + F); }

int sage_narrow_bwd_groups(const SnBwdPtrs* g, float* const* dwdb, int ng, int ldy, int n, int F, int act, int normalize, int mode, double count,
                           int lda, int fin, int ldd, hipStream_t st) {
  if (F <= 0 || fin <= 0) return 0;
  if (F > 32 || fin > 32 || ng < 1 || ng > 2) return CGC_EINVAL;
  for (int i = 0; i < ng; ++i)
    if (g[i].ws == nullptr || dwdb[i] == nullptr || (g[i].dagg != nullptr && ldd < fin)) return CGC_EINVAL;
  const int width = fin * F + F;
  if (n <= 0) {
    for (int i = 0; i < ng; ++i) (void)hipMemsetAsync(dwdb[i], 0, sizeof(float) * width, st);
    return 0;
  }
  const int tiles = ceil_div(n, 32), grid = sn_grid(n);
  const float inv_count = (float)(1.0 / count);
  const int fs = (F + 1) / 2;
  const SnBwdPtrs& g1 = g[ng - 1];
#define SN_LAUNCH(FS_, ACT_)                                                                                                       \
  hipLaunchKernelGGL((k_sage_narrow_bwd<FS_, ACT_>), dim3(grid, ng), dim3(256), 0, st, g[0], g1, ldy, n, F, act, normalize, mode, inv_count, \
                     lda, fin, ldd, tiles)
#define SN_ACT(FS_)                                                                                        \
  switch (act) {                                                                                           \
    case CGC_ACT_RELU: SN_LAUNCH(FS_, CGC_ACT_RELU); break;                                                \
    case CGC_ACT_ELU: SN_LAUNCH(FS_, CGC_ACT_ELU); break;                                                  \
    case CGC_ACT_LEAKYRELU: SN_LAUNCH(FS_, CGC_ACT_LEAKYRELU); break;                                      \
    default: SN_LAUNCH(FS_, CGC_ACT_IDENTITY); break;                                                      \
  }
  if (fs <= 8) { SN_ACT(8); } else if (fs <= 10) { SN_ACT(10); } else { SN_ACT(16); }
#undef SN_ACT
#undef SN_LAUNCH
  CGC_RETURN_IF_LAUNCH_FAILED();
  return launch_reduce_slots_f32_pair(g[0].ws, dwdb[0], g1.ws, dwdb[ng - 1], ng, grid, width, st);
}

extern "C" int cgc_sage_narrow_bwd(const float* dy, int ldy, const float* hn, const float* rinv, int n, int F, int act, int normalize,
                                   int mode, const float* mean, const float* istd, const float* gamma, const float* sums, double count,
                                   const float* agg, int lda, int fin, const float* W, float* dagg, int ldd, float* dwdb, float* ws,
                                   cgc_stream_t stream_) {
  const SnBwdPtrs g{dy, hn, rinv, mean, istd, gamma, sums, agg, W, dagg, ws};
  float* const out[1] = {dwdb};
  return sage_narrow_bwd_groups(&g, out, 1, ldy, n, F, act, normalize, mode, count, lda, fin, ldd, as_stream(stream_));
}

template <int KS, int ACT>
__global__ __launch_bounds__(256) void k_sage_narrow_fwd(const SnFwdPtrs p0, const SnFwdPtrs p1, int lda, int n, int K, int F, int normalize,
                                                         int , int tiles) {
  const bool second = blockIdx.y != 0;
  const float* __restrict__ agg = second ? p1.agg : p0.agg;
  const float* __restrict__ W = second ? p1.W : p0.W;
  const float* __restrict__ bias = second ? p1.bias : p0.bias;
  float* __restrict__ hn = second ? p1.hn : p0.hn;
  float* __restrict__ rinv_out = second ? p1.rinv : p0.rinv;
  float* __restrict__ ws = second ? p1.ws : p0.ws;
  __shared__ double xch[4][2][32];
  const int lane = threadIdx.x & 63, wave = threadIdx.x >> 6;
  const int f = lane & 31, half = lane >> 5;
  const bool fok = f < F;
  float bw[KS];
#pragma unroll
  for (int s = 0; s < KS; ++s) {
    const int k = 2 * s + half;
    bw[s] = (fok && k < K) ? W[(size_t)k * F + f] : 0.f;
  }
  const float bia = (fok && bias != nullptr) ? bias[f] : 0.f;
  double s1 = 0.0, s2 = 0.0;
  for (int tile = blockIdx.x * 4 + wave; tile < tiles; tile += gridDim.x * 4) {
    const int row0 = tile * 32;
    const float* __restrict__ a = agg + (size_t)min(row0 + f, n - 1) * lda;
    float av[KS];
#pragma unroll
    for (int s = 0; s < KS; ++s) {
      const int k = 2 * s + half;
      const float ld = a[k < K ? k : 0];
      av[s] = k < K ? ld : 0.f;
    }
    floatx16 acc;
#pragma unroll
    for (int r = 0; r < 16; ++r) acc[r] = bia;
#pragma unroll
    for (int s = 0; s < KS; ++s) acc = __builtin_amdgcn_mfma_f32_32x32x2f32(av[s], bw[s], acc, 0, 0, 0);
    float vv[16], rr[16];
#pragma unroll
    for (int r = 0; r < 16; ++r) {
      float v = fok ? acc[r] : 0.f;
      float rin = 1.f;
      if (normalize) {
        const float q = half_sum(v * v);
        rin = 1.f / fmaxf(sqrtf(q), L2_EPS);
        v *= rin;
      }
      vv[r] = v;
      rr[r] = rin;
    }
    if (row0 + 32 <= n) {
      if (fok) {
#pragma unroll
        for (int r = 0; r < 16; ++r) {
          const int row = row0 + (r & 3) + 8 * (r >> 2) + 4 * half;
          const double o = (double)act_fwd(vv[r], ACT);
          s1 += o;
          s2 = fma(o, o, s2);
          hn[(size_t)row * F + f] = vv[r];
        }
      }
      if (f == 0) {
#pragma unroll
        for (int r = 0; r < 16; ++r) rinv_out[row0 + (r & 3) + 8 * (r >> 2) + 4 * half] = rr[r];
      }
    } else {
#pragma unroll
      for (int r = 0; r < 16; ++r) {
        const int row = row0 + (r & 3) + 8 * (r >> 2) + 4 * half;
        if (row < n) {
          if (fok) {
            const double o = (double)act_fwd(vv[r], ACT);
            s1 += o;
            s2 = fma(o, o, s2);
            hn[(size_t)row * F + f] = vv[r];
          }
          if (f == 0) rinv_out[row] = rr[r];
        }
      }
    }
  }
  if (ws == nullptr) return;
  s1 += __shfl_xor(s1, 32);
  s2 += __shfl_xor(s2, 32);
  if (half == 0) { xch[wave][0][f] = s1; xch[wave][1][f] = s2; }
  __syncthreads();
  if (wave == 0 && half == 0 && fok) {
    double* __restrict__ slot = reinterpret_cast<double*>(ws) + (size_t)blockIdx.x * 2 * F;
    slot[f] = (xch[0][0][f] + xch[1][0][f]) + (xch[2][0][f] + xch[3][0][f]);
    slot[F + f] = (xch[0][1][f] + xch[1][1][f]) + (xch[2][1][f] + xch[3][1][f]);
  }
}

extern "C" int cgc_stats_blocks(int n, int F);
int sage_narrow_fwd_groups(const SnFwdPtrs* g, const SnFwdBn* bn, int ng, int lda, int n, int K, int F, int normalize, int act, int stats,
                           double count, hipStream_t st) {
  if (F <= 0) return 0;
  if (K <= 0 || K > 32 || F > 32 || ng < 1 || ng > 2) return CGC_EINVAL;
  for (int i = 0; i < ng; ++i)
    if (stats && (g[i].ws == nullptr || bn[i].mean == nullptr || bn[i].istd == nullptr)) return CGC_EINVAL;
  int slots = 0;
  if (n > 0) {
    const int tiles = ceil_div(n, 32);
    int grid = ceil_div(tiles, 4);
    const int cap = cgc_stats_blocks(n, F);
    if (grid > 1024) grid = 1024;
    if (stats && grid > cap) grid = cap > 0 ? cap : 1;
    SnFwdPtrs a0 = g[0], a1 = g[ng - 1];
    if (!stats) a0.ws = a1.ws = nullptr;
    const int ks = (K + 1) / 2;
#define SNF_LAUNCH(KS_, ACT_) \
  hipLaunchKernelGGL((k_sage_narrow_fwd<KS_, ACT_>), dim3(grid, ng), dim3(256), 0, st, a0, a1, lda, n, K, F, normalize, act, tiles)
#define SNF_ACT(KS_)                                                                                       \
  switch (act) {                                                                                           \
    case CGC_ACT_RELU: SNF_LAUNCH(KS_, CGC_ACT_RELU); break;                                               \
    case CGC_ACT_ELU: SNF_LAUNCH(KS_, CGC_ACT_ELU); break;                                                 \
    case CGC_ACT_LEAKYRELU: SNF_LAUNCH(KS_, CGC_ACT_LEAKYRELU); break;                                     \
    default: SNF_LAUNCH(KS_, CGC_ACT_IDENTITY); break;                                                     \
  }
    if (ks <= 8) { SNF_ACT(8); } else if (ks <= 10) { SNF_ACT(10); } else { SNF_ACT(16); }
#undef SNF_ACT
#undef SNF_LAUNCH
    CGC_RETURN_IF_LAUNCH_FAILED();
    slots = grid;
  }
  if (stats) {
    StatsFinPtrs f[2];
    for (int i = 0; i < ng; ++i)
      f[i] = StatsFinPtrs{g[i].ws, bn[i].running_mean, bn[i].running_var, bn[i].mean, bn[i].istd, reinterpret_cast<long long*>(bn[i].nbt),
                          bn[i].eps, bn[i].momentum};
    return launch_stats_finalize_groups(f, ng, slots, F, count, st);
  }
  return 0;
}

extern "C" int cgc_sage_narrow_fwd(const float* agg, int lda, const float* W, const float* bias, int n, int K, int F, int normalize,
                                   int act, float* hn, float* rinv, int stats, float* ws, double count, float eps, float momentum,
                                   float* running_mean, float* running_var, int64_t* num_batches_tracked, float* mean, float* istd,
                                   cgc_stream_t stream_) {
  const SnFwdPtrs g{agg, W, bias, hn, rinv, ws};
  const SnFwdBn bn{eps, momentum, running_mean, running_var, num_batches_tracked, mean, istd};
  return sage_narrow_fwd_groups(&g, &bn, 1, lda, n, K, F, normalize, act, stats, count, as_stream(stream_));
}
```

Before: 2808.

## Fold per-block slot reductions into producer kernels via last-block ticket

Column-reduction kernels (BN stats forward, BN backward reduce, colsum, softmax backward, sage-narrow fwd/bwd) now take a global atomic ticket. The last block to finish folds all per-block partial slots and writes the final sums or BN statistics, so the separate reduce or finalize kernel launches are dropped when the slot buffer is small. This removes a kernel launch and a dependency gap per reduction. In exchange it adds an atomic, a fence, agent-scope stores, a serial tail in a single block, and extra LDS reservation.

Result: no change. 2789 (-0.7%).

```diff
diff --git a/cgc-net_amd/csrc/fold.hpp b/cgc-net_amd/csrc/fold.hpp
--- /dev/null
+++ b/cgc-net_amd/csrc/fold.hpp
@@ -0,0 +1,124 @@
+#pragma once
+#include <atomic>
+
+#include "common.hpp"
+#include "groups.hpp"
+
+#define RS_GROUPS 32
+#define FOLD_TICKETS 256
+#define FOLD_MAX_BYTES (64 * 1024)
+
+#define FOLD_DEFINE_TICKETS()                                                      \
+  static __device__ unsigned int g_fold_tickets[FOLD_TICKETS];                     \
+  static std::atomic<unsigned> g_fold_next{0};                                     \
+  static inline int fold_take_tickets(int ny) {                                    \
+    return (int)(g_fold_next.fetch_add((unsigned)ny, std::memory_order_relaxed) % (FOLD_TICKETS - 1)); \
+  }
+
+static inline bool fold_fits(int slots, int width, size_t elem) { return (size_t)slots * (size_t)width * elem <= FOLD_MAX_BYTES; }
+#define FOLD_LDS_BYTES (sizeof(double) * RS_GROUPS * 32 + 16)
+
+__device__ __forceinline__ void slot_store(float* p, float v) { __hip_atomic_store(p, v, __ATOMIC_RELAXED, __HIP_MEMORY_SCOPE_AGENT); }
+__device__ __forceinline__ void slot_store(double* p, double v) { __hip_atomic_store(p, v, __ATOMIC_RELAXED, __HIP_MEMORY_SCOPE_AGENT); }
+
+__device__ __forceinline__ bool fold_is_last(unsigned int* ticket, unsigned int total, int* flag) {
+  asm volatile("s_waitcnt vmcnt(0)" ::: "memory");
+  __syncthreads();
+  if (threadIdx.x == 0) {
+    const unsigned int drawn = __hip_atomic_fetch_add(ticket, 1u, __ATOMIC_RELAXED, __HIP_MEMORY_SCOPE_AGENT);
+    const bool last = drawn + 1u == total;
+    if (last) {
+      __hip_atomic_store(ticket, 0u, __ATOMIC_RELAXED, __HIP_MEMORY_SCOPE_AGENT);
+      __builtin_amdgcn_fence(__ATOMIC_ACQUIRE, "agent");
+      asm volatile("s_waitcnt vmcnt(0)" ::: "memory");
+    }
+    *flag = last ? 1 : 0;
+  }
+  __syncthreads();
+  return *flag != 0;
+}
+
+template <typename IN>
+__device__ __forceinline__ double fold_column(const IN* col, bool ok, int slots, size_t stride, double (*part)[32]) {
+  const int cl = threadIdx.x & 31, g8 = threadIdx.x >> 5;
+  double a[4][4];
+#pragma unroll
+  for (int p = 0; p < 4; ++p)
+#pragma unroll
+    for (int u = 0; u < 4; ++u) a[p][u] = 0.0;
+  if (ok) {
+    for (int r0 = 0; r0 + g8 < slots; r0 += 4 * RS_GROUPS) {
+      IN v[4][4];
+#pragma unroll
+      for (int p = 0; p < 4; ++p)
+#pragma unroll
+        for (int u = 0; u < 4; ++u) {
+          const int k = r0 + g8 + 8 * p + RS_GROUPS * u;
+          v[p][u] = col[(size_t)(k < slots ? k : slots - 1) * stride];
+        }
+#pragma unroll
+      for (int p = 0; p < 4; ++p) {
+        const int k0 = r0 + g8 + 8 * p;
+        if (k0 + 3 * RS_GROUPS < slots) {
+#pragma unroll
+          for (int u = 0; u < 4; ++u) a[p][u] += (double)v[p][u];
+        } else {
+#pragma unroll
+          for (int u = 0; u < 4; ++u)
+            if (k0 + RS_GROUPS * u < slots) a[p][0] += (double)v[p][u];
+        }
+      }
+    }
+  }
+#pragma unroll
+  for (int p = 0; p < 4; ++p) part[g8 + 8 * p][cl] = (a[p][0] + a[p][1]) + (a[p][2] + a[p][3]);
+  __syncthreads();
+  double t[4] = {0.0, 0.0, 0.0, 0.0};
+  if (g8 == 0) {
+#pragma unroll
+    for (int g = 0; g < RS_GROUPS; g += 4) { t[0] += part[g][cl]; t[1] += part[g + 1][cl]; t[2] += part[g + 2][cl]; t[3] += part[g + 3][cl]; }
+  }
+  __syncthreads();
+  return (t[0] + t[1]) + (t[2] + t[3]);
+}
+
+template <typename OUT, typename IN>
+__device__ __forceinline__ void fold_slots(const IN* ws, int slots, int width, OUT* out, double (*part)[32]) {
+  const int cl = threadIdx.x & 31, g8 = threadIdx.x >> 5;
+  for (int c0 = 0; c0 < width; c0 += 32) {
+    const int c = c0 + cl;
+    const double s = fold_column(ws + c, c < width, slots, (size_t)width, part);
+    if (g8 == 0 && c < width) out[c] = (OUT)s;
+  }
+}
+
+__device__ __forceinline__ void fold_float_slots(const float* ws, int width, float* out, unsigned int* ticket, void* lds) {
+  double(*part)[32] = reinterpret_cast<double(*)[32]>(lds);
+  int* flag = reinterpret_cast<int*>(part + RS_GROUPS);
+  if (fold_is_last(ticket, gridDim.x, flag)) fold_slots<float, float>(ws, (int)gridDim.x, width, out, part);
+}
+
+__device__ __forceinline__ void stats_finalize_column(const StatsFinPtrs& p, int f, double s0, double s1, double count) {
+  const double m = s0 / count;
+  double var = s1 / count - m * m;
+  if (var < 0.0) var = 0.0;
+  p.mean[f] = (float)m;
+  p.istd[f] = (float)(1.0 / sqrt(var + (double)p.eps));
+  if (p.running_mean != nullptr) {
+    const double unbiased = var * count / (count > 1.0 ? count - 1.0 : 1.0);
+    p.running_mean[f] = (1.f - p.momentum) * p.running_mean[f] + p.momentum * (float)m;
+    p.running_var[f] = (1.f - p.momentum) * p.running_var[f] + p.momentum * (float)unbiased;
+  }
+}
+
+__device__ __forceinline__ void fold_stats_finalize(const StatsFinPtrs& p, int slots, int F, double count, double (*part)[32]) {
+  const double* ws = reinterpret_cast<const double*>(p.ws);
+  const int cl = threadIdx.x & 31, g8 = threadIdx.x >> 5;
+  if (threadIdx.x == 0 && p.nbt != nullptr) *p.nbt += 1;
+  for (int f0 = 0; f0 < F; f0 += 32) {
+    const int f = f0 + cl;
+    const double s0 = fold_column(ws + f, f < F, slots, 2 * (size_t)F, part);
+    const double s1 = fold_column(ws + F + f, f < F, slots, 2 * (size_t)F, part);
+    if (g8 == 0 && f < F) stats_finalize_column(p, f, s0, s1, count);
+  }
+}
diff --git a/cgc-net_amd/csrc/rowops.hip b/cgc-net_amd/csrc/rowops.hip
--- a/cgc-net_amd/csrc/rowops.hip
+++ b/cgc-net_amd/csrc/rowops.hip
@@ -1,11 +1,15 @@
+#include <algorithm>
 #include <type_traits>
 
 #include "common.hpp"
+#include "fold.hpp"
 #include "groups.hpp"
 
 #define L2_EPS 1e-12f
 #define RENORM_EPS 1e-15f
 #define MAX_SLOTS 1024
+
+FOLD_DEFINE_TICKETS()
 
 template <int VEC, int MAXJ, int NQ>
 __device__ __forceinline__ void col_reduce_store(float (&acc)[NQ][MAXJ][VEC], int F, int lpr, float* smem, float* slot) {
@@ -40,7 +44,7 @@
           if (c < F) {
             float t = acc[q][j][v];
             for (int w = 0; w < 3; ++w) t += smem[(w * NQ + q) * F + c];
-            slot[q * F + c] = t;
+            slot_store(slot + q * F + c, t);
           }
         }
   }
@@ -76,14 +80,13 @@
           if (c < F) {
             double t = acc[q][j][v];
             for (int w = 0; w < 3; ++w) t += smem[w * F + c];
-            slot[q * F + c] = t;
+            slot_store(slot + q * F + c, t);
           }
         }
     }
   }
 }
 
-#define RS_GROUPS 32
 template <typename OUT, typename IN = float>
 __global__ __launch_bounds__(32 * RS_GROUPS) void k_reduce_slots(const IN* __restrict__ ws, int slots, int width, OUT* __restrict__ out) {
   __shared__ double part[RS_GROUPS][32];
@@ -140,12 +143,6 @@
 }
 int launch_reduce_slots_f32_pair(const float* ws0, float* out0, const float* ws1, float* out1, int ng, int slots, int width, hipStream_t stream) {
   hipLaunchKernelGGL(k_reduce_slots_pair, dim3(ceil_div(width, 32), ng), dim3(32 * RS_GROUPS), 0, stream, ws0, out0, ws1, out1, slots, width);
-  CGC_RETURN_IF_LAUNCH_FAILED();
-  return 0;
-}
-
-int launch_reduce_slots_f32(const float* ws, int slots, int width, float* out, hipStream_t stream) {
-  hipLaunchKernelGGL(k_reduce_slots<float>, REDUCE_SLOTS_GRID(width), dim3(32 * RS_GROUPS), 0, stream, ws, slots, width, out);
   CGC_RETURN_IF_LAUNCH_FAILED();
   return 0;
 }
@@ -236,7 +233,8 @@
 template <int VEC, int MAXJ>
 __global__ __launch_bounds__(256) void k_l2norm_act_stats(const float* __restrict__ h, int n, int F, int lpr, int normalize,
                                                           int act, float* __restrict__ hn, float* __restrict__ rinv,
-                                                          float* __restrict__ ws) {
+                                                          float* __restrict__ ws, double* stats_out, const StatsFinPtrs fin,
+                                                          double count, int tk ) {
   extern __shared__ __attribute__((aligned(16))) float smem[];
   const RowGroup rg(lpr);
   double acc[2][MAXJ][VEC];
@@ -280,8 +278,15 @@
     }
     if (valid && rg.sl == 0) rinv[row] = r;
   }
-  if (ws != nullptr)
-    col_reduce_store_f64<VEC, MAXJ>(acc, F, lpr, reinterpret_cast<double*>(smem), reinterpret_cast<double*>(ws) + (size_t)blockIdx.x * 2 * F);
+  if (ws == nullptr) return;
+  col_reduce_store_f64<VEC, MAXJ>(acc, F, lpr, reinterpret_cast<double*>(smem), reinterpret_cast<double*>(ws) + (size_t)blockIdx.x * 2 * F);
+  if (tk < 0) return;
+  double(*part)[32] = reinterpret_cast<double(*)[32]>(smem);
+  if (!fold_is_last(&g_fold_tickets[tk], gridDim.x, reinterpret_cast<int*>(part + RS_GROUPS))) return;
+  if (stats_out != nullptr)
+    fold_slots<double, double>(reinterpret_cast<const double*>(ws), (int)gridDim.x, 2 * F, stats_out, part);
+  else
+    fold_stats_finalize(fin, (int)gridDim.x, F, count, part);
 }
 
 extern "C" int cgc_l2norm_act_stats(const float* h, int n, int F, int normalize, int act, float* hn, float* rinv,
@@ -295,10 +300,12 @@
   if (!cfg.ok) return CGC_EINVAL;
   float* wsp = stats ? ws : nullptr;
   if (stats && !ws) return CGC_EINVAL;
-  const size_t smem = sizeof(float) * 3 * 2 * F;
-  DISPATCH_COL(k_l2norm_act_stats, cfg, smem, as_stream(stream), h, n, F, cfg.lpr, normalize, act, hn, rinv, wsp);
-  CGC_RETURN_IF_LAUNCH_FAILED();
-  if (stats) {
+  const bool fold = stats && fold_fits(cfg.blocks, 2 * F, sizeof(double));
+  const size_t smem = std::max(sizeof(float) * 3 * 2 * F, fold ? FOLD_LDS_BYTES : 0);
+  DISPATCH_COL(k_l2norm_act_stats, cfg, smem, as_stream(stream), h, n, F, cfg.lpr, normalize, act, hn, rinv, wsp, stats, StatsFinPtrs{}, 0.0,
+               fold ? fold_take_tickets(1) : -1);
+  CGC_RETURN_IF_LAUNCH_FAILED();
+  if (stats && !fold) {
     hipLaunchKernelGGL((k_reduce_slots<double, double>), REDUCE_SLOTS_GRID(2 * F), dim3(32 * RS_GROUPS), 0, as_stream(stream),
                        reinterpret_cast<const double*>(ws), cfg.blocks, 2 * F, stats);
     CGC_RETURN_IF_LAUNCH_FAILED();
@@ -352,11 +359,6 @@
 __global__ __launch_bounds__(32 * RS_GROUPS) void k_stats_finalize(const StatsFinPtrs p0, const StatsFinPtrs p1, int slots, int F, double count) {
   const StatsFinPtrs& p = blockIdx.y ? p1 : p0;
   const double* __restrict__ ws = reinterpret_cast<const double*>(p.ws);
-  const float eps = p.eps, momentum = p.momentum;
-  float* running_mean = p.running_mean;
-  float* running_var = p.running_var;
-  float* __restrict__ mean = p.mean;
-  float* __restrict__ istd = p.istd;
   long long* nbt = p.nbt;
   __shared__ double part[2][RS_GROUPS][32];
   const int cl = threadIdx.x & 31, grp = threadIdx.x >> 5;
@@ -387,16 +389,7 @@
 #pragma unroll
     for (int u = 0; u < 4; ++u) { t0[u] += part[0][g + u][cl]; t1[u] += part[1][g + u][cl]; }
   const double s0 = (t0[0] + t0[1]) + (t0[2] + t0[3]), s1 = (t1[0] + t1[1]) + (t1[2] + t1[3]);
-  const double m = s0 / count;
-  double var = s1 / count - m * m;
-  if (var < 0.0) var = 0.0;
-  mean[f] = (float)m;
-  istd[f] = (float)(1.0 / sqrt(var + (double)eps));
-  if (running_mean != nullptr) {
-    const double unbiased = var * count / (count > 1.0 ? count - 1.0 : 1.0);
-    running_mean[f] = (1.f - momentum) * running_mean[f] + momentum * (float)m;
-    running_var[f] = (1.f - momentum) * running_var[f] + momentum * (float)unbiased;
-  }
+  stats_finalize_column(p, f, s0, s1, count);
 }
 
 int launch_stats_finalize_groups(const StatsFinPtrs* g, int ng, int slots, int F, double count, hipStream_t stream) {
@@ -420,9 +413,13 @@
     const bool vec_ok = (F % 4 == 0) && aligned16(h) && aligned16(hn);
     ColCfg cfg = col_cfg(n, F, vec_ok);
     if (!cfg.ok) return CGC_EINVAL;
-    const size_t smem = sizeof(float) * 3 * 2 * F;
-    DISPATCH_COL(k_l2norm_act_stats, cfg, smem, as_stream(stream), h, n, F, cfg.lpr, normalize, act, hn, rinv, ws);
+    const bool fold = fold_fits(cfg.blocks, 2 * F, sizeof(double));
+    const size_t smem = std::max(sizeof(float) * 3 * 2 * F, fold ? FOLD_LDS_BYTES : 0);
+    const StatsFinPtrs fin{ws, running_mean, running_var, mean, istd, reinterpret_cast<long long*>(num_batches_tracked), eps, momentum};
+    DISPATCH_COL(k_l2norm_act_stats, cfg, smem, as_stream(stream), h, n, F, cfg.lpr, normalize, act, hn, rinv, ws, (double*)nullptr, fin, count,
+                 fold ? fold_take_tickets(1) : -1);
     CGC_RETURN_IF_LAUNCH_FAILED();
+    if (fold) return 0;
     slots = cfg.blocks;
   }
   return launch_stats_finalize(ws, slots, F, count, eps, momentum, running_mean, running_var, mean, istd, num_batches_tracked, as_stream(stream));
@@ -509,7 +506,8 @@
 }
 
 template <int VEC, int MAXJ>
-__global__ __launch_bounds__(256) void k_bn_bwd_reduce(const BnRedPtrs p0, const BnRedPtrs p1, int ldy, int n, int F, int lpr, int act) {
+__global__ __launch_bounds__(256) void k_bn_bwd_reduce(const BnRedPtrs p0, const BnRedPtrs p1, int ldy, int n, int F, int lpr, int act,
+                                                       float* sums0, float* sums1, int tk ) {
   const BnRedPtrs& p = blockIdx.y ? p1 : p0;
   const float* __restrict__ dy = p.dy;
   const float* __restrict__ hn = p.hn;
@@ -550,6 +548,7 @@
     }
   }
   col_reduce_store<VEC, MAXJ, 2>(acc, F, lpr, smem, ws + (size_t)blockIdx.x * 2 * F);
+  if (tk >= 0) fold_float_slots(ws, 2 * F, blockIdx.y ? sums1 : sums0, &g_fold_tickets[tk + (int)blockIdx.y], smem);
 }
 
 int bn_bwd_reduce_groups(const BnRedPtrs* g, float* const* sums, int ng, int ldy, int n, int F, int act, hipStream_t stream) {
@@ -563,9 +562,12 @@
   for (int i = 0; i < ng; ++i) vec_ok = vec_ok && aligned16(g[i].dy) && aligned16(g[i].hn);
   ColCfg cfg = col_cfg(n, F, vec_ok);
   if (!cfg.ok) return CGC_EINVAL;
-  const size_t smem = sizeof(float) * 3 * 2 * F;
-  DISPATCH_COL_Y(k_bn_bwd_reduce, cfg, ng, smem, stream, g[0], g[ng - 1], ldy, n, F, cfg.lpr, act);
-  CGC_RETURN_IF_LAUNCH_FAILED();
+  const bool fold = fold_fits(cfg.blocks, 2 * F, sizeof(float));
+  const size_t smem = std::max(sizeof(float) * 3 * 2 * F, fold ? FOLD_LDS_BYTES : 0);
+  DISPATCH_COL_Y(k_bn_bwd_reduce, cfg, ng, smem, stream, g[0], g[ng - 1], ldy, n, F, cfg.lpr, act, sums[0], sums[ng - 1],
+                 fold ? fold_take_tickets(ng) : -1);
+  CGC_RETURN_IF_LAUNCH_FAILED();
+  if (fold) return 0;
   return launch_reduce_slots_f32_pair(g[0].ws, sums[0], g[ng - 1].ws, sums[ng - 1], ng, cfg.blocks, 2 * F, stream);
 }
 extern "C" int cgc_bn_bwd_reduce(const float* dy, int ldy, const float* hn, int n, int F, int act, const float* mean,
@@ -581,7 +583,8 @@
                                                        int normalize, int mode, const float* __restrict__ mean,
                                                        const float* __restrict__ istd, const float* __restrict__ gamma,
                                                        const float* __restrict__ sums, float inv_count, float* __restrict__ dh,
-                                                       float* __restrict__ ws ) {
+                                                       float* __restrict__ ws ,
+                                                       float* colsum_out, int tk ) {
   extern __shared__ __attribute__((aligned(16))) float smem[];
   const RowGroup rg(lpr);
   float csum[1][MAXJ][VEC];
@@ -707,7 +710,9 @@
       default: rows(std::integral_constant<int, CGC_ACT_IDENTITY>(), std::false_type()); break;
     }
   }
-  if (ws != nullptr) col_reduce_store<VEC, MAXJ, 1>(csum, F, lpr, smem, ws + (size_t)blockIdx.x * F);
+  if (ws == nullptr) return;
+  col_reduce_store<VEC, MAXJ, 1>(csum, F, lpr, smem, ws + (size_t)blockIdx.x * F);
+  if (tk >= 0) fold_float_slots(ws, F, colsum_out, &g_fold_tickets[tk], smem);
 }
 
 extern "C" int cgc_bn_act_l2_bwd(const float* dy, int ldy, const float* hn, const float* rinv, int n, int F, int act,
@@ -724,11 +729,12 @@
   if (!cfg.ok) return CGC_EINVAL;
   if (dh_colsum == nullptr) cfg.blocks = row_blocks(n, cfg.lpr);
   const float inv_count = (float)(1.0 / count);
-  const size_t smem = sizeof(float) * (3 + 5) * F;
+  const bool fold = dh_colsum && fold_fits(cfg.blocks, F, sizeof(float));
+  const size_t smem = std::max(sizeof(float) * (3 + 5) * F, fold ? FOLD_LDS_BYTES : 0);
   DISPATCH_COL(k_bn_act_l2_bwd, cfg, smem, as_stream(stream), dy, ldy, hn, rinv, n, F, cfg.lpr, act, normalize, mode, mean, istd,
-               gamma, sums, inv_count, dh, dh_colsum ? ws : (float*)nullptr);
-  CGC_RETURN_IF_LAUNCH_FAILED();
-  if (dh_colsum) {
+               gamma, sums, inv_count, dh, dh_colsum ? ws : (float*)nullptr, dh_colsum, fold ? fold_take_tickets(1) : -1);
+  CGC_RETURN_IF_LAUNCH_FAILED();
+  if (dh_colsum && !fold) {
     hipLaunchKernelGGL(k_reduce_slots<float>, REDUCE_SLOTS_GRID(F), dim3(32 * RS_GROUPS), 0, as_stream(stream), ws, cfg.blocks, F, dh_colsum);
     CGC_RETURN_IF_LAUNCH_FAILED();
   }
@@ -736,7 +742,8 @@
 }
 
 template <int VEC, int MAXJ>
-__global__ __launch_bounds__(256) void k_colsum(const float* __restrict__ x, int ld, int n, int F, int lpr, float* __restrict__ ws) {
+__global__ __launch_bounds__(256) void k_colsum(const float* __restrict__ x, int ld, int n, int F, int lpr, float* __restrict__ ws, float* out,
+                                                int tk ) {
   extern __shared__ __attribute__((aligned(16))) float smem[];
   const RowGroup rg(lpr);
   float acc[1][MAXJ][VEC];
@@ -760,6 +767,7 @@
     }
   }
   col_reduce_store<VEC, MAXJ, 1>(acc, F, lpr, smem, ws + (size_t)blockIdx.x * F);
+  if (tk >= 0) fold_float_slots(ws, F, out, &g_fold_tickets[tk], smem);
 }
 
 extern "C" int cgc_colsum(const float* x, int ld, int n, int F, float* out, float* ws, cgc_stream_t stream) {
@@ -771,9 +779,11 @@
   const bool vec_ok = (F % 4 == 0) && (ld % 4 == 0) && aligned16(x);
   ColCfg cfg = col_cfg(n, F, vec_ok);
   if (!cfg.ok) return CGC_EINVAL;
-  const size_t smem = sizeof(float) * 3 * F;
-  DISPATCH_COL(k_colsum, cfg, smem, as_stream(stream), x, ld, n, F, cfg.lpr, ws);
-  CGC_RETURN_IF_LAUNCH_FAILED();
+  const bool fold = fold_fits(cfg.blocks, F, sizeof(float));
+  const size_t smem = std::max(sizeof(float) * 3 * F, fold ? FOLD_LDS_BYTES : 0);
+  DISPATCH_COL(k_colsum, cfg, smem, as_stream(stream), x, ld, n, F, cfg.lpr, ws, out, fold ? fold_take_tickets(1) : -1);
+  CGC_RETURN_IF_LAUNCH_FAILED();
+  if (fold) return 0;
   hipLaunchKernelGGL(k_reduce_slots<float>, REDUCE_SLOTS_GRID(F), dim3(32 * RS_GROUPS), 0, as_stream(stream), ws, cfg.blocks, F, out);
   CGC_RETURN_IF_LAUNCH_FAILED();
   return 0;
@@ -865,7 +875,8 @@
 
 template <int VEC, int MAXJ>
 __global__ __launch_bounds__(256) void k_softmax_bwd(const float* __restrict__ S, const float* __restrict__ dS, int n, int C,
-                                                     int ld, int lpr, float* __restrict__ dx, float* __restrict__ ws) {
+                                                     int ld, int lpr, float* __restrict__ dx, float* __restrict__ ws, float* colsum_out,
+                                                     int tk ) {
   extern __shared__ __attribute__((aligned(16))) float smem[];
   const RowGroup rg(lpr);
   float csum[1][MAXJ][VEC];
@@ -909,7 +920,9 @@
       }
     }
   }
-  if (ws != nullptr) col_reduce_store<VEC, MAXJ, 1>(csum, C, lpr, smem, ws + (size_t)blockIdx.x * C);
+  if (ws == nullptr) return;
+  col_reduce_store<VEC, MAXJ, 1>(csum, C, lpr, smem, ws + (size_t)blockIdx.x * C);
+  if (tk >= 0) fold_float_slots(ws, C, colsum_out, &g_fold_tickets[tk], smem);
 }
 
 extern "C" int cgc_softmax_fwd(const float* x, int n, int C, int ld, float* out, cgc_stream_t stream) {
@@ -946,10 +959,12 @@
   ColCfg cfg = col_cfg(n, C, vec);
   if (!cfg.ok) return CGC_EINVAL;
   if (dx_colsum == nullptr) cfg.blocks = row_blocks(n, cfg.lpr);
-  const size_t smem = dx_colsum ? sizeof(float) * 3 * C : 0;
-  DISPATCH_COL(k_softmax_bwd, cfg, smem, as_stream(stream), S, dS, n, C, ld, cfg.lpr, dx, dx_colsum ? ws : (float*)nullptr);
-  CGC_RETURN_IF_LAUNCH_FAILED();
-  if (dx_colsum) {
+  const bool fold = dx_colsum && fold_fits(cfg.blocks, C, sizeof(float));
+  const size_t smem = dx_colsum ? std::max(sizeof(float) * 3 * C, fold ? FOLD_LDS_BYTES : 0) : 0;
+  DISPATCH_COL(k_softmax_bwd, cfg, smem, as_stream(stream), S, dS, n, C, ld, cfg.lpr, dx, dx_colsum ? ws : (float*)nullptr, dx_colsum,
+               fold ? fold_take_tickets(1) : -1);
+  CGC_RETURN_IF_LAUNCH_FAILED();
+  if (dx_colsum && !fold) {
     hipLaunchKernelGGL(k_reduce_slots<float>, REDUCE_SLOTS_GRID(C), dim3(32 * RS_GROUPS), 0, as_stream(stream), ws, cfg.blocks, C, dx_colsum);
     CGC_RETURN_IF_LAUNCH_FAILED();
   }
diff --git a/cgc-net_amd/csrc/sagenarrow.hip b/cgc-net_amd/csrc/sagenarrow.hip
--- a/cgc-net_amd/csrc/sagenarrow.hip
+++ b/cgc-net_amd/csrc/sagenarrow.hip
@@ -1,8 +1,11 @@
 #include "common.hpp"
+#include "fold.hpp"
 #include "groups.hpp"
 
 #define L2_EPS 1e-12f
 typedef float floatx16 __attribute__((ext_vector_type(16)));
+
+FOLD_DEFINE_TICKETS()
 
 template <int CTRL>
 __device__ __forceinline__ float dpp_step(float v) {
@@ -20,7 +23,8 @@
 
 template <int FS, int ACT>
 __global__ __launch_bounds__(256) void k_sage_narrow_bwd(const SnBwdPtrs p0, const SnBwdPtrs p1, int ldy, int n, int F, int ,
-                                                         int normalize, int mode, float inv_count, int lda, int fin, int ldd, int tiles) {
+                                                         int normalize, int mode, float inv_count, int lda, int fin, int ldd, int tiles,
+                                                         float* dwdb0, float* dwdb1, int tk ) {
   const bool second = blockIdx.y != 0;
   const float* __restrict__ dy = second ? p1.dy : p0.dy;
   const float* __restrict__ hn = second ? p1.hn : p0.hn;
@@ -33,7 +37,7 @@
   const float* __restrict__ W = second ? p1.W : p0.W;
   float* __restrict__ dagg = second ? p1.dagg : p0.dagg;
   float* __restrict__ ws = second ? p1.ws : p0.ws;
-  __shared__ float strip[4][17 * 64];
+  __shared__ __attribute__((aligned(16))) float strip[4][17 * 64];
   const int lane = threadIdx.x & 63, wave = threadIdx.x >> 6;
   const int f = lane & 31, half = lane >> 5;
   const bool fok = f < F;
@@ -126,15 +130,15 @@
     for (int r = 0; r < 16; ++r) {
       const float v = (xch[(0 * 17 + r) * 64 + lane] + xch[(1 * 17 + r) * 64 + lane]) + (xch[(2 * 17 + r) * 64 + lane] + xch[(3 * 17 + r) * 64 + lane]);
       const int k = (r & 3) + 8 * (r >> 2) + 4 * half;
-      if (fok && k < fin) slot[k * F + f] = v;
+      if (fok && k < fin) slot_store(slot + k * F + f, v);
     }
     float d = (xch[(0 * 17 + 16) * 64 + lane] + xch[(1 * 17 + 16) * 64 + lane]) + (xch[(2 * 17 + 16) * 64 + lane] + xch[(3 * 17 + 16) * 64 + lane]);
     d += __shfl_xor(d, 32);
-    if (fok && half == 0) slot[fin * F + f] = d;
-  }
-}
-
-int launch_reduce_slots_f32(const float* ws, int slots, int width, float* out, hipStream_t stream);
+    if (fok && half == 0) slot_store(slot + fin * F + f, d);
+  }
+  static_assert(sizeof(strip) >= FOLD_LDS_BYTES, "the fold's scratch does not fit the strips");
+  if (tk >= 0) fold_float_slots(ws, fin * F + F, second ? dwdb1 : dwdb0, &g_fold_tickets[tk + (int)blockIdx.y], &strip[0][0]);
+}
 
 static int sn_grid(int n) {
   const int tiles = ceil_div(n, 32);
@@ -159,9 +163,11 @@
   const float inv_count = (float)(1.0 / count);
   const int fs = (F + 1) / 2;
   const SnBwdPtrs& g1 = g[ng - 1];
+  const bool fold = fold_fits(grid, width, sizeof(float));
+  const int tk = fold ? fold_take_tickets(ng) : -1;
 #define SN_LAUNCH(FS_, ACT_)                                                                                                       \
   hipLaunchKernelGGL((k_sage_narrow_bwd<FS_, ACT_>), dim3(grid, ng), dim3(256), 0, st, g[0], g1, ldy, n, F, act, normalize, mode, inv_count, \
-                     lda, fin, ldd, tiles)
+                     lda, fin, ldd, tiles, dwdb[0], dwdb[ng - 1], tk)
 #define SN_ACT(FS_)                                                                                        \
   switch (act) {                                                                                           \
     case CGC_ACT_RELU: SN_LAUNCH(FS_, CGC_ACT_RELU); break;                                                \
@@ -173,6 +179,7 @@
 #undef SN_ACT
 #undef SN_LAUNCH
   CGC_RETURN_IF_LAUNCH_FAILED();
+  if (fold) return 0;
   return launch_reduce_slots_f32_pair(g[0].ws, dwdb[0], g1.ws, dwdb[ng - 1], ng, grid, width, st);
 }
 
@@ -187,7 +194,8 @@
 
 template <int KS, int ACT>
 __global__ __launch_bounds__(256) void k_sage_narrow_fwd(const SnFwdPtrs p0, const SnFwdPtrs p1, int lda, int n, int K, int F, int normalize,
-                                                         int , int tiles) {
+                                                         int , int tiles, const StatsFinPtrs f0, const StatsFinPtrs f1, double count,
+                                                         int tk ) {
   const bool second = blockIdx.y != 0;
   const float* __restrict__ agg = second ? p1.agg : p0.agg;
   const float* __restrict__ W = second ? p1.W : p0.W;
@@ -195,7 +203,8 @@
   float* __restrict__ hn = second ? p1.hn : p0.hn;
   float* __restrict__ rinv_out = second ? p1.rinv : p0.rinv;
   float* __restrict__ ws = second ? p1.ws : p0.ws;
-  __shared__ double xch[4][2][32];
+  __shared__ double lds[RS_GROUPS + 1][32];
+  double(*xch)[2][32] = reinterpret_cast<double(*)[2][32]>(&lds[0][0]);
   const int lane = threadIdx.x & 63, wave = threadIdx.x >> 6;
   const int f = lane & 31, half = lane >> 5;
   const bool fok = f < F;
@@ -273,9 +282,12 @@
   __syncthreads();
   if (wave == 0 && half == 0 && fok) {
     double* __restrict__ slot = reinterpret_cast<double*>(ws) + (size_t)blockIdx.x * 2 * F;
-    slot[f] = (xch[0][0][f] + xch[1][0][f]) + (xch[2][0][f] + xch[3][0][f]);
-    slot[F + f] = (xch[0][1][f] + xch[1][1][f]) + (xch[2][1][f] + xch[3][1][f]);
-  }
+    slot_store(slot + f, (xch[0][0][f] + xch[1][0][f]) + (xch[2][0][f] + xch[3][0][f]));
+    slot_store(slot + F + f, (xch[0][1][f] + xch[1][1][f]) + (xch[2][1][f] + xch[3][1][f]));
+  }
+  if (tk < 0) return;
+  if (fold_is_last(&g_fold_tickets[tk + (int)blockIdx.y], gridDim.x, reinterpret_cast<int*>(&lds[RS_GROUPS][0])))
+    fold_stats_finalize(second ? f1 : f0, (int)gridDim.x, F, count, lds);
 }
 
 extern "C" int cgc_stats_blocks(int n, int F);
@@ -286,6 +298,11 @@
   for (int i = 0; i < ng; ++i)
     if (stats && (g[i].ws == nullptr || bn[i].mean == nullptr || bn[i].istd == nullptr)) return CGC_EINVAL;
   int slots = 0;
+  StatsFinPtrs f[2];
+  for (int i = 0; i < ng; ++i)
+    f[i] = stats ? StatsFinPtrs{g[i].ws, bn[i].running_mean, bn[i].running_var, bn[i].mean, bn[i].istd, reinterpret_cast<long long*>(bn[i].nbt),
+                                bn[i].eps, bn[i].momentum}
+                 : StatsFinPtrs{};
   if (n > 0) {
     const int tiles = ceil_div(n, 32);
     int grid = ceil_div(tiles, 4);
@@ -295,8 +312,10 @@
     SnFwdPtrs a0 = g[0], a1 = g[ng - 1];
     if (!stats) a0.ws = a1.ws = nullptr;
     const int ks = (K + 1) / 2;
+    const bool fold = stats && fold_fits(grid, 2 * F, sizeof(double));
+    const int tk = fold ? fold_take_tickets(ng) : -1;
 #define SNF_LAUNCH(KS_, ACT_) \
-  hipLaunchKernelGGL((k_sage_narrow_fwd<KS_, ACT_>), dim3(grid, ng), dim3(256), 0, st, a0, a1, lda, n, K, F, normalize, act, tiles)
+  hipLaunchKernelGGL((k_sage_narrow_fwd<KS_, ACT_>), dim3(grid, ng), dim3(256), 0, st, a0, a1, lda, n, K, F, normalize, act, tiles, f[0], f[ng - 1], count, tk)
 #define SNF_ACT(KS_)                                                                                       \
   switch (act) {                                                                                           \
     case CGC_ACT_RELU: SNF_LAUNCH(KS_, CGC_ACT_RELU); break;                                               \
@@ -308,15 +327,10 @@
 #undef SNF_ACT
 #undef SNF_LAUNCH
     CGC_RETURN_IF_LAUNCH_FAILED();
+    if (fold) return 0;
     slots = grid;
   }
-  if (stats) {
-    StatsFinPtrs f[2];
-    for (int i = 0; i < ng; ++i)
-      f[i] = StatsFinPtrs{g[i].ws, bn[i].running_mean, bn[i].running_var, bn[i].mean, bn[i].istd, reinterpret_cast<long long*>(bn[i].nbt),
-                          bn[i].eps, bn[i].momentum};
-    return launch_stats_finalize_groups(f, ng, slots, F, count, st);
-  }
+  if (stats) return launch_stats_finalize_groups(f, ng, slots, F, count, st);
   return 0;
 }
 
```
